# dcy0577/Enhancing-3D-Point-Cloud-Segmentation-Using-Multi-Modal-Fusion-with-2D-Images

Measured on AMD Instinct MI355X. Metric: input points/s through MV-KPConv KPFCNN forward+backward (pyramid + fusion + fwd + bwd + SGD), higher is better.
Workload: dtype f32; 1 GPU; early_fusion_kpfcnn5_sphere19k_x1_per_gpu; views=3, parallelism=dp1, execution=hipGraph[net|chain|enc2d(x2 every 2nd step)+fa], ranks=1, input_lookahead_batches=2, capacity_overflow=False

## Files before the change

enhancing-3d-point-cloud-segmentation-using-multi-modal-fusion-with-2d-images_amd/_lib.py:

```python
import ctypes as C
import os
import re

_HERE = os.path.dirname(os.path.abspath(__file__))
LIB_PATH = os.path.join(_HERE, "libmvkpconv.so")
HEADER_PATH = os.path.join(_HERE, "..", "include", "mvkpconv.h")
SCENE_HEADER_PATH = os.path.join(_HERE, "..", "include", "mvkpconv_scene.h")
TRAIN_HEADER_PATH = os.path.join(_HERE, "..", "include", "mvkpconv_train.h")
SPHERE_HEADER_PATH = os.path.join(_HERE, "..", "include", "mvkpconv_sphere.h")

CTYPES = {"int": C.c_int, "int32_t": C.c_int32, "int64_t": C.c_int64, "float": C.c_float, "double": C.c_double,
          "const char*": C.c_char_p}
_SCALARS = frozenset(t for t in CTYPES if not t.endswith("*"))
_POINTEES = _SCALARS | {"void", "char", "uint8_t", "uint16_t"}
_INTEGER = r"-?(?:0[xX][0-9a-fA-F]+|0|[1-9][0-9]*)"
_DIRECTIVE = re.compile(r"\s*#\s*(?:include\s*<[\w./]+>|ifdef\s+__cplusplus|ifndef\s+\w+_H|endif"
                        r"|define\s+(\w+)(?:\s+(%s))?)\s*" % _INTEGER)
_STRUCT = re.compile(r"typedef\s+struct(?:\s+\w+)?\s*\{([^{}]*)\}\s*(mvk_\w+)\s*;")
_FUNCTION = re.compile(r"([\w\s*]+?)\b(mvk_\w+)\s*\(([^(){};]*)\)\s*;")


def parse_header(text):
    functions, structs, constants = {}, {}, {}

    def fail(pos, what):
        pos += len(text[pos:]) - len(text[pos:].lstrip())
        raise ValueError("mvkpconv.h line %d: %s" % (text.count("\n", 0, pos) + 1, what))

    def canonical(pos, spelling):
        tokens = re.findall(r"\w+|\S", spelling)
        const = tokens[:1] == ["const"]
        base, stars = "".join(tokens[const:const + 1]), tokens[const + 1:]
        if not (stars == [] and not const and base in _SCALARS
                or stars == ["*"] and (base in _POINTEES or base in structs)):
            fail(pos, "unsupported type %r" % " ".join(tokens))
        return "const " * const + base + "*" * len(stars)

    def declarator(pos, spelling):
        m = re.fullmatch(r"(.*[\s*])([A-Za-z_]\w*)\s*", spelling, re.S)
        if not m or m.group(2) == "const" or m.group(2) in _POINTEES:
            fail(pos, "expected '<type> <name>', found %r" % spelling.strip())
        return canonical(pos, m.group(1)), m.group(2)

    text = re.sub(r"/\*.*?\*/|//[^\n]*", lambda m: " " + "\n" * m.group().count("\n"), text, flags=re.S)
    lines = text.split("\n")
    for i, line in enumerate(lines):
        if line.lstrip().startswith("#"):
            m = _DIRECTIVE.fullmatch(line)
            name, value = m.groups() if m else (None, None)
            if not m or (name is not None and (name.startswith("MVK_") != (value is not None) or name in constants)):
                raise ValueError("mvkpconv.h line %d: unsupported preprocessor line %r" % (i + 1, line.strip()))
            if value is not None:
                constants[name] = int(value, 0)
            lines[i] = ""
    text = "\n".join(lines)

    block = re.fullmatch(r'\s*extern\s+"C"\s*\{(.*)\}\s*', text, re.S)
    if not block:
        fail(0, 'expected one extern "C" { ... } block around all declarations')
    pos, end = block.start(1), block.end(1)
    while True:
        pos = re.compile(r"\s*").match(text, pos, end).end()
        if pos == end:
            return functions, structs, constants
        s = _STRUCT.match(text, pos, end)
        f = None if s else _FUNCTION.match(text, pos, end)
        if (s or f) and (s or f).group(2) in functions.keys() | structs.keys():
            fail(pos, "%s is declared twice" % (s or f).group(2))
        if s:
            fields, at = [], s.start(1)
            *statements, tail = s.group(1).split(";")
            if tail.strip() or not statements:
                fail(s.end(1) - len(tail), "struct %s: expected 'type name;' fields" % s.group(2))
            for statement in statements:
                first, *more = statement.split(",")
                ctype, name = declarator(at, first)
                if more and (ctype.endswith("*") or not all(re.fullmatch(r"\s*[A-Za-z_]\w*\s*", n) for n in more)):
                    fail(at, "only scalar fields share a declaration, found %r" % statement.strip())
                fields += [(ctype, n.strip()) for n in [name] + more]
                at += len(statement) + 1
            structs[s.group(2)] = tuple(fields)
        elif f:
            params, at = [], f.start(3)
            for spelling in f.group(3).split(",") if f.group(3).strip() != "void" else ():
                params.append(declarator(at, spelling))
                at += len(spelling) + 1
            functions[f.group(2)] = (canonical(pos, f.group(1)), tuple(params))
        else:
            fail(pos, "neither a function declaration nor a struct typedef: %r" % text[pos:end].split("\n")[0].strip())
        pos = (s or f).end()


def _bind(functions, structs):
    classes = {}

    def ctype(t):
        if t in CTYPES:
            return CTYPES[t]
        assert t.endswith("*"), t
        pointee = t[6 * t.startswith("const "):-1]
        return C.POINTER(classes[pointee]) if pointee in classes else C.c_void_p

    for name, fields in structs.items():
        classes[name] = type("".join(w.capitalize() for w in name.split("_")[1:]), (C.Structure,),
                             {"_fields_": [(n, ctype(t)) for t, n in fields], "__doc__": name + " (include/mvkpconv.h)"})
    return classes, {name: (ctype(ret), [ctype(t) for t, _ in params]) for name, (ret, params) in functions.items()}


def _read_header(path=None, name="mvkpconv.h"):
    path = HEADER_PATH if path is None else path
    if not os.path.exists(path):
        raise RuntimeError(
            "include/%s is not there (%s). The binding reads every prototype of libmvkpconv.so from it -- "
            "run the package from a checkout of the repository; there is no second copy of the C ABI." % (name, path))
    with open(path) as f:
        return f.read()


FUNCTIONS, STRUCTS, CONSTANTS = parse_header(_read_header())
_CLASSES, _PROTOTYPES = _bind(FUNCTIONS, STRUCTS)
EXPORTS = tuple(FUNCTIONS)
ABI_VERSION = CONSTANTS["MVK_ABI_VERSION"]

SCENE_FUNCTIONS, _scene_structs, SCENE_CONSTANTS = parse_header(_read_header(SCENE_HEADER_PATH, "mvkpconv_scene.h"))
if _scene_structs or SCENE_FUNCTIONS.keys() & FUNCTIONS.keys() or SCENE_CONSTANTS.keys() & CONSTANTS.keys():
    raise ValueError("mvkpconv_scene.h: it may declare neither a struct nor a name of mvkpconv.h")
_SCENE_PROTOTYPES = _bind(SCENE_FUNCTIONS, {})[1]

TRAIN_FUNCTIONS, _train_structs, TRAIN_CONSTANTS = parse_header(_read_header(TRAIN_HEADER_PATH, "mvkpconv_train.h"))
if (_train_structs or TRAIN_FUNCTIONS.keys() & (FUNCTIONS.keys() | SCENE_FUNCTIONS.keys())
        or TRAIN_CONSTANTS.keys() & (CONSTANTS.keys() | SCENE_CONSTANTS.keys())):
    raise ValueError("mvkpconv_train.h: it may declare neither a struct nor a name of the other two headers")
_TRAIN_PROTOTYPES = _bind(TRAIN_FUNCTIONS, {})[1]

SPHERE_FUNCTIONS, _sphere_structs, SPHERE_CONSTANTS = parse_header(_read_header(SPHERE_HEADER_PATH, "mvkpconv_sphere.h"))
if (_sphere_structs
        or SPHERE_FUNCTIONS.keys() & (FUNCTIONS.keys() | SCENE_FUNCTIONS.keys() | TRAIN_FUNCTIONS.keys())
        or SPHERE_CONSTANTS.keys() & (CONSTANTS.keys() | SCENE_CONSTANTS.keys() | TRAIN_CONSTANTS.keys())):
    raise ValueError("mvkpconv_sphere.h: it may declare neither a struct nor a name of the other three headers")
_SPHERE_PROTOTYPES = _bind(SPHERE_FUNCTIONS, {})[1]
BnFwdProblem, BnBwdProblem = _CLASSES["mvk_bn_fwd_problem"], _CLASSES["mvk_bn_bwd_problem"]
BnFinish, ATransform = _CLASSES["mvk_bn_finish"], _CLASSES["mvk_a_transform"]
RevList, RegLayer = _CLASSES["mvk_rev_list"], _CLASSES["mvk_reg_layer"]

_lib = None
_owner_pid = None

FORK_MESSAGE = ("the MV-KPConv HIP library was initialised in process %d and is being called from its forked child %d: "
                "a HIP context does not survive fork(). Start DataLoader workers with multiprocessing_context='spawn', "
                "or let the workers emit only stacked points / lengths and build the pyramid "
                "(datasets.common.segmentation_inputs_sphere) in the main process -- see INTEGRATION.md")


def _check_process():
    pid = os.getpid()
    if _owner_pid is not None and pid != _owner_pid:
        raise RuntimeError(FORK_MESSAGE % (_owner_pid, pid))
    try:
        import torch
        if torch.cuda._is_in_bad_fork():
            raise RuntimeError(FORK_MESSAGE % (os.getppid(), pid))
    except (ImportError, AttributeError):
        pass


def lib():
    global _lib, _owner_pid
    _check_process()
    if _lib is None:
        if not os.path.exists(LIB_PATH):
            raise RuntimeError(
                "libmvkpconv.so is not built (%s). Run `python __graft_entry__.py build` -- there is "
                "no CPU fallback for the MV-KPConv hot path." % LIB_PATH)
        l = C.CDLL(LIB_PATH)
        for name, (res, args) in list(_PROTOTYPES.items()) + list(_SCENE_PROTOTYPES.items()) + list(_TRAIN_PROTOTYPES.items()) \
                + list(_SPHERE_PROTOTYPES.items()):
            fn = getattr(l, name)
            fn.restype = res
            fn.argtypes = args
        if l.mvk_abi_version() != ABI_VERSION:
            raise RuntimeError("libmvkpconv.so ABI %d != expected %d; rebuild" % (l.mvk_abi_version(), ABI_VERSION))
        _lib = l
        _owner_pid = os.getpid()
    return _lib


def check(rc):
    if rc != 0:
        raise RuntimeError(lib().mvk_last_error().decode("utf-8", "replace"))
```

enhancing-3d-point-cloud-segmentation-using-multi-modal-fusion-with-2d-images_amd/build.py:

```python
import os
import subprocess
import sys

HERE = os.path.dirname(os.path.abspath(__file__))
CSRC = os.path.join(HERE, "csrc")
OUT = os.path.join(HERE, "libmvkpconv.so")
ARCH = "gfx950"

SOURCES = [
    ("error.cpp", []),
    ("kpconv.hip", []),
    ("gemm.hip", []),
    ("gemm32s.hip", []),
    ("pool.hip", []),
    ("bn.hip", []),
    ("optim.hip", []),
    ("deform.hip", []),
    ("loss.hip", []),
    ("batchpad.hip", []),
    ("revlist.hip", []),
    ("subsample.hip", ["-ffp-contract=off"]),
    ("neighbors.hip", ["-ffp-contract=off"]),
    ("fusion.hip", ["-ffp-contract=off"]),
    ("vote.hip", ["-ffp-contract=off"]),
    ("pn2.hip", ["-ffp-contract=off"]),
    ("chunk.hip", ["-ffp-contract=off"]),
    ("pn2_ordered.hip", ["-ffp-contract=off"]),
    ("pn2_mlp.hip", ["-ffp-contract=off"]),
    ("pn2_rows.hip", ["-ffp-contract=off"]),
    ("scene_inputs.hip", ["-ffp-contract=off"]),
    ("train_inputs.hip", ["-ffp-contract=off"]),
    ("sphere_inputs.hip", ["-ffp-contract=off"]),
]


def _hipcc():
    for c in (os.environ.get("HIPCC"), "/opt/rocm/bin/hipcc", "hipcc"):
        if c and (os.path.isabs(c) and os.path.exists(c) or not os.path.isabs(c)):
            return c
    return "hipcc"


def _stale(target, deps):
    if not os.path.exists(target):
        return True
    t = os.path.getmtime(target)
    return any(os.path.getmtime(d) > t for d in deps if os.path.exists(d))


def build_library(force=False, verbose=False):
    hipcc = _hipcc()
    common = [os.path.join(CSRC, "common.h"), os.path.join(CSRC, "blockscan.h"), os.path.join(CSRC, "compact.h"),
              os.path.join(CSRC, "pn2_rows.h"), os.path.join(CSRC, "unproject.h"), os.path.join(CSRC, "select_frames.h"),
              os.path.join(CSRC, "knn_core.h"), os.path.join(HERE, "..", "include", "mvkpconv_sphere.h"),
              os.path.join(HERE, "..", "include", "mvkpconv.h"), os.path.join(HERE, "..", "include", "mvkpconv_scene.h"),
              os.path.join(HERE, "..", "include", "mvkpconv_train.h"),
              os.path.join(HERE, "..", "include", "mvk_prime_list.h"), os.path.abspath(__file__)]
    objs, jobs = [], []
    for src, extra in SOURCES:
        sp = os.path.join(CSRC, src)
        if not os.path.exists(sp):
            raise FileNotFoundError(sp)
        obj = os.path.join(CSRC, os.path.splitext(src)[0] + ".o")
        if force or _stale(obj, [sp] + common):
            cmd = [hipcc, "--offload-arch=" + ARCH, "-O3", "-std=c++17", "-fPIC", "-c", sp, "-o", obj] + extra
            if src.endswith(".cpp"):
                cmd = [hipcc, "-O2", "-std=c++17", "-fPIC", "-c", sp, "-o", obj]
            jobs.append(cmd)
        objs.append(obj)
    if jobs:
        from concurrent.futures import ThreadPoolExecutor
        n = max(1, min(int(os.environ.get("MVK_BUILD_JOBS", "6")), os.cpu_count() or 1, len(jobs)))

        def run(cmd):
            if verbose:
                print(" ".join(cmd), flush=True)
            subprocess.check_call(cmd)
        with ThreadPoolExecutor(n) as pool:
            list(pool.map(run, jobs))
    if force or _stale(OUT, objs):
        cmd = [hipcc, "--offload-arch=" + ARCH, "-shared", "-fPIC", "-o", OUT] + objs
        if verbose:
            print(" ".join(cmd))
        subprocess.check_call(cmd)
    return OUT


if __name__ == "__main__":
    print(build_library(force="--force" in sys.argv, verbose=True))
```

enhancing-3d-point-cloud-segmentation-using-multi-modal-fusion-with-2d-images_amd/csrc/gemm.hip:

```cpp
#include <stdlib.h>

#include <mutex>
#include <type_traits>

#include "common.h"

namespace {

typedef float f32x4 __attribute__((ext_vector_type(4)));

constexpr int BK = 32;

template <bool CONTIG_K, int ROWS>
struct Tile {
  static constexpr int LD = CONTIG_K ? 40 : ROWS + 4;
  static constexpr int FLOATS = CONTIG_K ? ROWS * 40 : BK * (ROWS + 4);
  static constexpr int NF4 = ROWS * BK / 4;
  static constexpr int NV = (NF4 + 255) / 256;
  static constexpr int IPT = ROWS / 4;
  float4 v[NV];

  __device__ __forceinline__ void transform(const float* __restrict__ xs, int64_t k0, int64_t kbase0, int64_t i0, int64_t imax,
                                            int64_t kmax, int64_t nvalid, float slope, float* __restrict__ out, int64_t ld,
                                            int tid) {
    static_assert(CONTIG_K, "the transform is written for k-contiguous A tiles");
#pragma unroll
    for (int u = 0; u < NV; ++u) {
      const int f = tid + 256 * u;
      if (NF4 % 256 == 0 || f < NF4) {
        const int i = f >> 3, kq = (f & 7) * 4;
        const int64_t gi = i0 + i, gk = k0 + kq;
        const float* t = xs + (gk - kbase0) * 4;
        float e[4] = {v[u].x, v[u].y, v[u].z, v[u].w};
#pragma unroll
        for (int c = 0; c < 4; ++c) {
          const float4 q = *reinterpret_cast<const float4*>(t + 4 * c);
          float z = (e[c] - q.x) * q.y + q.z;
          z = z > 0.f ? z : z * slope;
          e[c] = gi < nvalid ? z : 0.f;
        }
        v[u] = make_float4(e[0], e[1], e[2], e[3]);
        if (out && gi < imax) {
          float* o = out + gi * ld + gk;
          if (gk + 3 < kmax && (ld & 3) == 0)
            *reinterpret_cast<float4*>(o) = v[u];
          else {
#pragma unroll
            for (int c = 0; c < 4; ++c)
              if (gk + c < kmax) o[c] = e[c];
          }
        }
      }
    }
  }

  __device__ __forceinline__ void load(const float* __restrict__ src, int64_t ld, int64_t i0, int64_t imax,
                                       int64_t k0, int64_t kmax, int vec, int tid) {
#pragma unroll
    for (int u = 0; u < NV; ++u) {
      float t[4] = {0.f, 0.f, 0.f, 0.f};
      const int f = tid + 256 * u;
      if (NF4 % 256 == 0 || f < NF4) {
        if (CONTIG_K) {
          const int i = f >> 3, kq = (f & 7) * 4;
          const int64_t gi = i0 + i, gk = k0 + kq;
          if (gi < imax) {
            const float* p = src + gi * ld + gk;
            if (vec == 4 && gk + 3 < kmax) {
              const float4 q = *reinterpret_cast<const float4*>(p);
              t[0] = q.x; t[1] = q.y; t[2] = q.z; t[3] = q.w;
            } else if (vec == 2 && gk + 3 < kmax) {
              const float2 q0 = *reinterpret_cast<const float2*>(p), q1 = *reinterpret_cast<const float2*>(p + 2);
              t[0] = q0.x; t[1] = q0.y; t[2] = q1.x; t[3] = q1.y;
            } else {
#pragma unroll
              for (int e = 0; e < 4; ++e)
                if (gk + e < kmax) t[e] = p[e];
            }
          }
        } else {
          const int k = f / IPT, iq = (f % IPT) * 4;
          const int64_t gk = k0 + k, gi = i0 + iq;
          if (gk < kmax) {
            const float* p = src + gk * ld + gi;
            if (vec == 4 && gi + 3 < imax) {
              const float4 q = *reinterpret_cast<const float4*>(p);
              t[0] = q.x; t[1] = q.y; t[2] = q.z; t[3] = q.w;
            } else if (vec == 2 && gi + 3 < imax) {
              const float2 q0 = *reinterpret_cast<const float2*>(p), q1 = *reinterpret_cast<const float2*>(p + 2);
              t[0] = q0.x; t[1] = q0.y; t[2] = q1.x; t[3] = q1.y;
            } else {
#pragma unroll
              for (int e = 0; e < 4; ++e)
                if (gi + e < imax) t[e] = p[e];
            }
          }
        }
      }
      v[u] = make_float4(t[0], t[1], t[2], t[3]);
    }
  }

  template <int VEC>
  __device__ __forceinline__ void load_fast(const float* __restrict__ src, int64_t ld, int64_t i0, int64_t imax,
                                            int64_t k0, int tid) {
#pragma unroll
    for (int u = 0; u < NV; ++u) {
      int f = tid + 256 * u;
      if (NF4 % 256 != 0) f = f < NF4 ? f : NF4 - 1;
      const float* p;
      if (CONTIG_K) {
        const int i = f >> 3, kq = (f & 7) * 4;
        int64_t gi = i0 + i;
        gi = gi < imax ? gi : imax - 1;
        p = src + gi * ld + (k0 + kq);
      } else {
        const int k = f / IPT, iq = (f % IPT) * 4;
        int64_t gi = i0 + iq;
        gi = gi + 3 < imax ? gi : imax - 4;
        p = src + (k0 + k) * ld + gi;
      }
      if (VEC == 4) {
        const f32x4 q = *reinterpret_cast<const f32x4*>(p);
        v[u] = make_float4(q[0], q[1], q[2], q[3]);
      } else {
        const float2 q0 = *reinterpret_cast<const float2*>(p), q1 = *reinterpret_cast<const float2*>(p + 2);
        v[u] = make_float4(q0.x, q0.y, q1.x, q1.y);
      }
    }
  }

  static __device__ __forceinline__ bool fast_ok(int64_t imax, int vec) {
    return CONTIG_K ? (vec >= 2 && imax >= 1) : (vec == 4 && imax >= 4 && (imax & 3) == 0);
  }

  template <int VEC>
  __device__ __forceinline__ void fetch(const float* __restrict__ src, int64_t ld, int64_t i0, int64_t imax, int64_t k0,
                                        int64_t kmax, int vec, int tid) {
    if (VEC == 0)
      load(src, ld, i0, imax, k0, kmax, vec, tid);
    else
      load_fast<VEC>(src, ld, i0, imax, k0, tid);
  }

  __device__ __forceinline__ void store(float* __restrict__ T, int tid) const {
#pragma unroll
    for (int u = 0; u < NV; ++u) {
      const int f = tid + 256 * u;
      if (NF4 % 256 == 0 || f < NF4) {
        const f32x4 q = {v[u].x, v[u].y, v[u].z, v[u].w};
        if (CONTIG_K) {
          const int i = f >> 3, kq = (f & 7) * 4;
          *reinterpret_cast<f32x4*>(&T[i * LD + kq]) = q;
        } else {
          const int k = f / IPT, iq = (f % IPT) * 4;
          *reinterpret_cast<f32x4*>(&T[k * LD + iq]) = q;
        }
      }
    }
  }

  static __device__ __forceinline__ f32x4 frag(const float* __restrict__ T, int r0, int j, int lane) {
    const int i = lane & 15, g = lane >> 4;
    if (CONTIG_K) {
      return *reinterpret_cast<const f32x4*>(&T[(r0 + i) * LD + 16 * j + 4 * g]);
    } else {
      f32x4 r;
      const float* p = &T[(16 * j + 4 * g) * LD + r0 + i];
      r[0] = p[0];
      r[1] = p[LD];
      r[2] = p[2 * LD];
      r[3] = p[3 * LD];
      return r;
    }
  }
};

struct GemmArgs {
  const float* A;
  const float* B;
  float* C;
  int64_t M, N, Kd, lda, ldb, k_per_split;
  int atomic_out, accumulate, vecA, vecB;
  float* bn_part;
  const int32_t* n_valid;
  const float* bias;
  float act_slope;
  const float* A2;
  const float* B2;
  int64_t Kd2, lda2, ldb2;
  int vecA2, vecB2;
  const void* sc_idx;
  int sc_idx64, sc_c1;
  int64_t sc_stride, sc_ns;
  float* sc_dst;
  float* sc_rest;
  float* det_ws;
  int* det_cnt;
  int det_gx, det_nsplit;
  int seg_shift;
  int64_t seg_extra;
  int* fin_cnt;
  int fin_gy;
  float fin_eps, fin_momentum;
  float* fin_mean;
  float* fin_invstd;
  float* fin_rmean;
  float* fin_rvar;
  long long* fin_nbt;
  const float* ax_mean;
  const float* ax_invstd;
  const float* ax_gamma;
  const float* ax_beta;
  float ax_slope;
  const int32_t* ax_nvalid;
  float* ax_out;
};

constexpr int XF_KMAX = 512;

template <bool TA, bool TB, int PM, int QN, int WM, int WN, bool DUAL = false, bool XF = false>
__device__ __forceinline__ void gemm_body(const GemmArgs& a, const int bx, const int by, const int bz) {
  static_assert(WM * WN == 4, "four waves per workgroup");
  constexpr int TM = 16 * PM * WM, TN = 16 * QN * WN;
  typedef Tile<!TA, TM> TileA;
  typedef Tile<TB, TN> TileB;
  __shared__ __attribute__((aligned(16))) float lds[2 * (TileA::FLOATS + TileB::FLOATS)];
  __shared__ __attribute__((aligned(16))) float xs[XF ? 4 * (XF_KMAX + BK) : 4];
  float* const As = lds;
  float* const Bs = lds + 2 * TileA::FLOATS;
  const int tid = threadIdx.x, lane = tid & 63, wave = tid >> 6;
  const int wm = wave / WN, wn = wave % WN;
  const int64_t m0 = (int64_t)by * TM, n0 = (int64_t)bx * TN;
  const int64_t ktot = DUAL ? a.Kd + a.Kd2 : a.Kd;
  const int64_t kbeg_all = (int64_t)bz * a.k_per_split;
  const int64_t kend_all = kbeg_all + a.k_per_split < ktot ? kbeg_all + a.k_per_split : ktot;

  f32x4 acc[PM][QN];
#pragma unroll
  for (int p = 0; p < PM; ++p)
#pragma unroll
    for (int q = 0; q < QN; ++q) acc[p][q] = (f32x4){0.f, 0.f, 0.f, 0.f};

  int64_t x_nvalid = 0;
  if (XF) {
    for (int k = tid; k < XF_KMAX + BK; k += 256) {
      const int64_t gk = kbeg_all + k;
      float4 q = make_float4(0.f, 0.f, 0.f, 0.f);
      if (gk < a.Kd && k < a.k_per_split + BK) q = make_float4(a.ax_mean[gk], a.ax_invstd[gk] * a.ax_gamma[gk], a.ax_beta[gk], 0.f);
      *reinterpret_cast<float4*>(&xs[4 * k]) = q;
    }
    x_nvalid = a.ax_nvalid ? (int64_t)*a.ax_nvalid : a.M;
    __syncthreads();
  }
  float* const x_out = (XF && bx == 0) ? a.ax_out : nullptr;

  TileA la0, la1;
  TileB lb0, lb1;
  const int ra = wm * 16 * PM, rb = wn * 16 * QN;
  auto compute = [&](const float* __restrict__ Ta, const float* __restrict__ Tb) {
#pragma unroll
    for (int j = 0; j < 2; ++j) {
      f32x4 fa[PM], fb[QN];
#pragma unroll
      for (int p = 0; p < PM; ++p) fa[p] = TileA::frag(Ta, ra + 16 * p, j, lane);
#pragma unroll
      for (int q = 0; q < QN; ++q) fb[q] = TileB::frag(Tb, rb + 16 * q, j, lane);
#pragma unroll
      for (int s = 0; s < 4; ++s)
#pragma unroll
        for (int p = 0; p < PM; ++p)
#pragma unroll
          for (int q = 0; q < QN; ++q)
            acc[p][q] = __builtin_amdgcn_mfma_f32_16x16x4f32(fa[p][s], fb[q][s], acc[p][q], 0, 0, 0);
    }
  };
  float* const A0 = As;
  float* const A1 = As + TileA::FLOATS;
  float* const B0 = Bs;
  float* const B1 = Bs + TileB::FLOATS;
  auto run_range = [&](const float* __restrict__ pA, const int64_t lda, const int vecA, const float* __restrict__ pB,
                       const int64_t ldb, const int vecB, int64_t kbeg, const int64_t kend) {
  auto Bat = [&](const int64_t k) -> const float* {
    return (TB && !DUAL && a.seg_shift >= 0) ? pB + (k >> a.seg_shift) * a.seg_extra : pB;
  };
  auto putA = [&](TileA& la, float* __restrict__ T, const int64_t kt) {
    if constexpr (XF) la.transform(xs, kt, kbeg_all, m0, a.M, a.Kd, x_nvalid, a.ax_slope, x_out, lda, tid);
    la.store(T, tid);
  };
  auto pipeline = [&](auto va, auto vb, const int64_t klim) {
    constexpr int VA = decltype(va)::value, VB = decltype(vb)::value;
    if (kbeg >= klim) return;
    la0.template fetch<VA>(pA, lda, m0, a.M, kbeg, klim, vecA, tid);
    lb0.template fetch<VB>(Bat(kbeg), ldb, n0, a.N, kbeg, klim, vecB, tid);
    if (kbeg + BK < klim) {
      la1.template fetch<VA>(pA, lda, m0, a.M, kbeg + BK, klim, vecA, tid);
      lb1.template fetch<VB>(Bat(kbeg + BK), ldb, n0, a.N, kbeg + BK, klim, vecB, tid);
    }
    putA(la0, A0, kbeg);
    lb0.store(B0, tid);
    __syncthreads();
    for (int64_t k0 = kbeg; k0 < klim; k0 += 2 * BK) {
      if (k0 + 2 * BK < klim) {
        la0.template fetch<VA>(pA, lda, m0, a.M, k0 + 2 * BK, klim, vecA, tid);
        lb0.template fetch<VB>(Bat(k0 + 2 * BK), ldb, n0, a.N, k0 + 2 * BK, klim, vecB, tid);
      }
      compute(A0, B0);
      if (k0 + BK >= klim) break;
      putA(la1, A1, k0 + BK);
      lb1.store(B1, tid);
      __syncthreads();
      if (k0 + 3 * BK < klim) {
        la1.template fetch<VA>(pA, lda, m0, a.M, k0 + 3 * BK, klim, vecA, tid);
        lb1.template fetch<VB>(Bat(k0 + 3 * BK), ldb, n0, a.N, k0 + 3 * BK, klim, vecB, tid);
      }
      compute(A1, B1);
      if (k0 + 2 * BK >= klim) break;
      putA(la0, A0, k0 + 2 * BK);
      lb0.store(B0, tid);
      __syncthreads();
    }
  };
  const bool fastA = TileA::fast_ok(a.M, vecA), fastB = TileB::fast_ok(a.N, vecB);
  const int64_t kfull = kbeg + (kend - kbeg) / BK * BK;
  typedef std::integral_constant<int, 4> I4;
  typedef std::integral_constant<int, 2> I2;
  typedef std::integral_constant<int, 0> I0;
  if (fastA && fastB && vecA == 4 && vecB == 4) {
    pipeline(I4(), I4(), kfull);
  } else if (fastA && fastB && vecA == 2 && vecB == 4) {
    pipeline(I2(), I4(), kfull);
  } else {
    pipeline(I0(), I0(), kend);
    kbeg = kend;
  }
  if (kfull < kend && kbeg < kend) {
    __syncthreads();
    la0.load(pA, lda, m0, a.M, kfull, kend, vecA, tid);
    lb0.load(Bat(kfull), ldb, n0, a.N, kfull, kend, vecB, tid);
    putA(la0, A0, kfull);
    lb0.store(B0, tid);
    __syncthreads();
    compute(A0, B0);
  }
  };
  if (!DUAL) {
    run_range(a.A, a.lda, a.vecA, a.B, a.ldb, a.vecB, kbeg_all, kend_all);
  } else {
    if (kbeg_all < a.Kd) run_range(a.A, a.lda, a.vecA, a.B, a.ldb, a.vecB, kbeg_all, kend_all < a.Kd ? kend_all : a.Kd);
    if (kend_all > a.Kd) {
      if (kbeg_all < a.Kd) __syncthreads();
      run_range(a.A2, a.lda2, a.vecA2, a.B2, a.ldb2, a.vecB2, kbeg_all > a.Kd ? kbeg_all - a.Kd : 0, kend_all - a.Kd);
    }
  }

  if (a.det_ws) {
    constexpr int NB = PM * QN, SLOT = NB * 4 * 256;
    const int64_t tile = (int64_t)by * a.det_gx + bx;
    const __amdgpu_buffer_rsrc_t slots = park_rsrc(a.det_ws + tile * a.det_nsplit * SLOT);
    const uint32_t lane_off = (uint32_t)tid * 16u;
#pragma unroll
    for (int p = 0; p < PM; ++p)
#pragma unroll
      for (int q = 0; q < QN; ++q)
        park_store4(slots, (uint32_t)bz * (SLOT * 4u) + (uint32_t)(p * QN + q) * 4096u + lane_off, acc[p][q]);
    park_wait();
    __syncthreads();
    int* const flag = reinterpret_cast<int*>(lds);
    if (tid == 0) {
      const int old = __hip_atomic_fetch_add(a.det_cnt + tile, 1, __ATOMIC_RELAXED, __HIP_MEMORY_SCOPE_AGENT);
      const int last = old == a.det_nsplit - 1;
      if (last) __hip_atomic_store(a.det_cnt + tile, 0, __ATOMIC_RELAXED, __HIP_MEMORY_SCOPE_AGENT);
      *flag = last;
    }
    __syncthreads();
    const int last = *flag;
    __syncthreads();
    if (!last) return;
#pragma unroll
    for (int p = 0; p < PM; ++p)
#pragma unroll
      for (int q = 0; q < QN; ++q) acc[p][q] = (f32x4){0.f, 0.f, 0.f, 0.f};
    constexpr int ZC = NB >= 8 ? 2 : 4;
    for (int z0 = 0; z0 < a.det_nsplit; z0 += ZC) {
      f32x4 t[ZC][NB];
#pragma unroll
      for (int zz = 0; zz < ZC; ++zz) {
        const int z = z0 + zz < a.det_nsplit ? z0 + zz : a.det_nsplit - 1;
#pragma unroll
        for (int b = 0; b < NB; ++b) t[zz][b] = park_load4(slots, (uint32_t)z * (SLOT * 4u) + (uint32_t)b * 4096u + lane_off);
      }
#pragma unroll
      for (int zz = 0; zz < ZC; ++zz)
        if (z0 + zz < a.det_nsplit) {
#pragma unroll
          for (int p = 0; p < PM; ++p)
#pragma unroll
            for (int q = 0; q < QN; ++q) acc[p][q] += t[zz][p * QN + q];
        }
    }
  }

  const int ci = lane & 15, g4 = (lane >> 4) * 4;
#pragma unroll
  for (int q = 0; q < QN; ++q) {
    const int64_t col = n0 + rb + 16 * q + ci;
    if (col < a.N) {
      const float bq = a.bias ? a.bias[col] : 0.f;
#pragma unroll
      for (int p = 0; p < PM; ++p)
#pragma unroll
        for (int r = 0; r < 4; ++r) {
          const int64_t row = m0 + ra + 16 * p + g4 + r;
          if (row < a.M) {
            if (a.sc_idx) {
              const float v = acc[p][q][r];
              if (col < a.sc_c1) {
                const int j = a.sc_idx64 ? load_idx<true>(a.sc_idx, row * a.sc_stride, a.sc_ns)
                                         : load_idx<false>(a.sc_idx, row * a.sc_stride, a.sc_ns);
                if (j >= 0) atomicAdd(a.sc_dst + (int64_t)j * a.sc_c1 + col, v);
              } else {
                float* c2 = a.sc_rest + row * (a.N - a.sc_c1) + (col - a.sc_c1);
                if (a.atomic_out) atomicAdd(c2, v);
                else *c2 = v;
              }
              continue;
            }
            float* c = a.C + row * a.N + col;
            if (a.atomic_out)
              atomicAdd(c, acc[p][q][r]);
            else if (a.accumulate)
              *c += acc[p][q][r];
            else if (a.bias) {
              const float v = acc[p][q][r] + bq;
              *c = v > 0.f ? v : v * a.act_slope;
            } else
              *c = acc[p][q][r];
          }
        }
    }
  }

  if (a.bn_part) {
    int64_t nv = a.n_valid ? (int64_t)*a.n_valid : a.M;
    nv = nv < a.M ? nv : a.M;
    const int64_t wcnt = nv - (m0 + ra) < 0 ? 0 : (nv - (m0 + ra) > 16 * PM ? 16 * PM : nv - (m0 + ra));
    const int64_t bcnt = nv - m0 < 0 ? 0 : (nv - m0 > TM ? TM : nv - m0);
    const int64_t blk = m0 / TM;
    float* red = lds;
    const __amdgpu_buffer_rsrc_t part_rs = park_rsrc(a.bn_part);
    auto put_part = [&](const int64_t col, const float sum, const float m2) {
      if (a.fin_cnt) {
        park_store1(part_rs, (uint32_t)(((blk * 2) * a.N + col) * 4), sum);
        park_store1(part_rs, (uint32_t)(((blk * 2 + 1) * a.N + col) * 4), m2);
      } else {
        a.bn_part[(blk * 2) * a.N + col] = sum;
        a.bn_part[(blk * 2 + 1) * a.N + col] = m2;
      }
    };
    if (WM > 1) __syncthreads();
    float s[QN], mu[QN];
#pragma unroll
    for (int q = 0; q < QN; ++q) {
      s[q] = 0.f;
#pragma unroll
      for (int p = 0; p < PM; ++p)
#pragma unroll
        for (int r = 0; r < 4; ++r)
          if (16 * p + g4 + r < wcnt) s[q] += acc[p][q][r];
      s[q] += __shfl_xor(s[q], 16);
      s[q] += __shfl_xor(s[q], 32);
      if (WM > 1 && lane < 16) red[wm * TN + rb + 16 * q + ci] = s[q];
    }
    if (WM > 1) {
      __syncthreads();
#pragma unroll
      for (int q = 0; q < QN; ++q) {
        s[q] = 0.f;
#pragma unroll
        for (int w = 0; w < WM; ++w) s[q] += red[w * TN + rb + 16 * q + ci];
      }
    }
#pragma unroll
    for (int q = 0; q < QN; ++q) {
      mu[q] = bcnt > 0 ? s[q] / (float)bcnt : 0.f;
      float m2 = 0.f;
#pragma unroll
      for (int p = 0; p < PM; ++p)
#pragma unroll
        for (int r = 0; r < 4; ++r)
          if (16 * p + g4 + r < wcnt) {
            const float d = acc[p][q][r] - mu[q];
            m2 += d * d;
          }
      m2 += __shfl_xor(m2, 16);
      m2 += __shfl_xor(m2, 32);
      if (WM > 1) {
        if (lane < 16) red[(WM + wm) * TN + rb + 16 * q + ci] = m2;
      } else {
        const int64_t col = n0 + rb + 16 * q + ci;
        if (lane < 16 && col < a.N && m0 < a.M) put_part(col, s[q], m2);
      }
    }
    if (WM > 1) {
      __syncthreads();
      if (wm == 0 && lane < 16) {
#pragma unroll
        for (int q = 0; q < QN; ++q) {
          float m2 = 0.f;
#pragma unroll
          for (int w = 0; w < WM; ++w) m2 += red[(WM + w) * TN + rb + 16 * q + ci];
          const int64_t col = n0 + rb + 16 * q + ci;
          if (col < a.N && m0 < a.M) put_part(col, s[q], m2);
        }
      }
    }
    if (a.fin_cnt) {
      park_wait();
      __syncthreads();
      int* const flag = reinterpret_cast<int*>(lds);
      if (tid == 0) {
        const int old = __hip_atomic_fetch_add(a.fin_cnt + bx, 1, __ATOMIC_RELAXED, __HIP_MEMORY_SCOPE_AGENT);
        const int last = old == a.fin_gy - 1;
        if (last) __hip_atomic_store(a.fin_cnt + bx, 0, __ATOMIC_RELAXED, __HIP_MEMORY_SCOPE_AGENT);
        *flag = last;
      }
      __syncthreads();
      const int last = *flag;
      __syncthreads();
      if (!last) return;
      constexpr int C4 = TN / 4, BL = 256 / C4;
      const int c4 = tid % C4, bl = tid / C4;
      const int64_t col0 = n0 + 4 * c4;
      const int nb = nv > 0 ? (int)((nv + TM - 1) / TM) : 0;
      f32x4 X = {0.f, 0.f, 0.f, 0.f}, Y = {0.f, 0.f, 0.f, 0.f}, ref = {0.f, 0.f, 0.f, 0.f};
      if (col0 < a.N && nb > 0) {
        const float n0f = (float)(nv < TM ? nv : TM);
        ref = park_load4(part_rs, (uint32_t)(col0 * 4));
        ref = ref * (1.f / n0f);
        constexpr int FP = 4;
        for (int i0 = bl; i0 < nb; i0 += FP * BL) {
          f32x4 u[FP], w[FP];
#pragma unroll
          for (int t = 0; t < FP; ++t) {
            const int i = i0 + t * BL < nb ? i0 + t * BL : nb - 1;
            u[t] = park_load4(part_rs, (uint32_t)((((int64_t)i * 2) * a.N + col0) * 4));
            w[t] = park_load4(part_rs, (uint32_t)((((int64_t)i * 2 + 1) * a.N + col0) * 4));
          }
#pragma unroll
          for (int t = 0; t < FP; ++t)
            if (i0 + t * BL < nb) {
              const int64_t left = nv - (int64_t)(i0 + t * BL) * TM;
              const float ni = (float)(left < TM ? left : TM);
              const f32x4 d = u[t] * (1.f / ni) - ref;
              X += u[t];
              Y += w[t] + ni * d * d;
            }
        }
      }
      float* const q1 = lds;
      float* const q2 = lds + 256 * 4;
      *reinterpret_cast<f32x4*>(&q1[bl * TN + 4 * c4]) = X;
      *reinterpret_cast<f32x4*>(&q2[bl * TN + 4 * c4]) = Y;
      float* const qr = lds + 2 * 256 * 4;
      if (bl == 0) *reinterpret_cast<f32x4*>(&qr[4 * c4]) = ref;
      __syncthreads();
      const int64_t col = n0 + tid;
      if (tid < TN && col < a.N) {
        float x = 0.f, y = 0.f;
#pragma unroll 4
        for (int l = 0; l < BL; ++l) {
          x += q1[l * TN + tid];
          y += q2[l * TN + tid];
        }
        float mu = 0.f, var = 0.f, is = 0.f;
        if (nv > 0) {
          mu = x / (float)nv;
          const float dm = mu - qr[tid];
          float M2 = y - (float)nv * dm * dm;
          M2 = M2 > 0.f ? M2 : 0.f;
          var = M2 / (float)nv;
          is = rsqrtf(var + a.fin_eps);
        }
        a.fin_mean[col] = mu;
        a.fin_invstd[col] = is;
        if (a.fin_rmean && nv > 0) {
          const float unbiased = nv > 1 ? var * ((float)nv / (float)(nv - 1)) : var;
          a.fin_rmean[col] = (1.f - a.fin_momentum) * a.fin_rmean[col] + a.fin_momentum * mu;
          a.fin_rvar[col] = (1.f - a.fin_momentum) * a.fin_rvar[col] + a.fin_momentum * unbiased;
        }
      }
      if (a.fin_nbt && bx == 0 && tid == 0) *a.fin_nbt += 1;
    }
  }
}

template <bool TA, bool TB, int PM, int QN, int WM, int WN>
__global__ __launch_bounds__(256) void gemm_f32_mfma(const GemmArgs a) {
  gemm_body<TA, TB, PM, QN, WM, WN>(a, blockIdx.x, blockIdx.y, blockIdx.z);
}

template <bool TB, int PM>
__global__ __launch_bounds__(256) void gemm_f32_mfma_xf(const GemmArgs a) {
  gemm_body<false, TB, PM, 1, 1, 4, false, true>(a, blockIdx.x, blockIdx.y, blockIdx.z);
}

template <bool TA, bool TB, int PM, int QN, int WM, int WN>
__global__ __launch_bounds__(256) void gemm_f32_mfma_pair(const GemmArgs a0, const GemmArgs a1, int gx0, int gz0, int gz1) {
  if ((int)blockIdx.x < gx0) {
    if ((int)blockIdx.z >= gz0) return;
    gemm_body<TA, TB, PM, QN, WM, WN>(a0, blockIdx.x, blockIdx.y, blockIdx.z);
  } else {
    if ((int)blockIdx.z >= gz1) return;
    gemm_body<TA, TB, PM, QN, WM, WN>(a1, blockIdx.x - gx0, blockIdx.y, blockIdx.z);
  }
}

template <bool TA, bool TB, int PM, int QN, int WM, int WN>
__global__ __launch_bounds__(256) void gemm_f32_mfma_dual(const GemmArgs a) {
  gemm_body<TA, TB, PM, QN, WM, WN, true>(a, blockIdx.x, blockIdx.y, blockIdx.z);
}

struct GroupEntry {
  GemmArgs args;
  int gx, gy, gz;
  int wg_begin;
};

template <bool TA, bool TB, int PM, int QN, int WM, int WN>
__global__ __launch_bounds__(256) void gemm_f32_mfma_grouped(const GroupEntry* __restrict__ tab, int n_prob) {
  const int b = blockIdx.x;
  int lo = 0, hi = n_prob - 1;
  while (lo < hi) {
    const int mid = (lo + hi + 1) >> 1;
    if (tab[mid].wg_begin <= b)
      lo = mid;
    else
      hi = mid - 1;
  }
  const GroupEntry& e = tab[lo];
  const int local = b - e.wg_begin;
  const int bx = local % e.gx, by = (local / e.gx) % e.gy, bz = local / (e.gx * e.gy);
  GemmArgs a = e.args;
  a.A = load_global_ptr(&e.args.A);
  a.B = load_global_ptr(&e.args.B);
  a.C = load_global_ptr(&e.args.C);
  a.bn_part = load_global_ptr(&e.args.bn_part);
  a.n_valid = load_global_ptr(&e.args.n_valid);
  a.det_ws = load_global_ptr(&e.args.det_ws);
  a.det_cnt = load_global_ptr(&e.args.det_cnt);
  gemm_body<TA, TB, PM, QN, WM, WN>(a, bx, by, bz);
}


struct Plan {
  int pm, qn, narrow, split;
  int64_t tm() const { return narrow ? 64 * pm : 16 * pm; }
  int64_t tn() const { return narrow ? 16 * qn : 64 * qn; }
};

struct SplitArena {
  float* ws = nullptr;
  int* cnt = nullptr;
  int64_t ws_floats = 0, n_cnt = 0;
  int64_t ws_off = 0, cnt_off = 0;
  int64_t ws_top = 0, cnt_top = 0;
};
SplitArena g_arena;
std::mutex g_arena_mu;

bool ordered_splits() { return g_arena.ws != nullptr; }

int arena_take(hipStream_t st, int64_t tiles, int split, int64_t slot, float** ws, int** cnt) {
  const int64_t need = (tiles * split * slot + 63) / 64 * 64;
  std::lock_guard<std::mutex> lock(g_arena_mu);
  if (need > g_arena.ws_floats || tiles > g_arena.n_cnt) return 1;
  hipStreamCaptureStatus cap = hipStreamCaptureStatusNone;
  if (hipStreamIsCapturing(st, &cap) != hipSuccess) {
    (void)hipGetLastError();
    cap = hipStreamCaptureStatusNone;
  }
  if (cap != hipStreamCaptureStatusNone) {
    if (g_arena.ws_top - need < g_arena.ws_off || g_arena.cnt_top - tiles < g_arena.cnt_off) return 2;
    g_arena.ws_top -= need;
    g_arena.cnt_top -= tiles;
    *ws = g_arena.ws + g_arena.ws_top;
    *cnt = g_arena.cnt + g_arena.cnt_top;
    return 0;
  }
  const int64_t ws_cap = g_arena.ws_top < g_arena.ws_floats / 4 ? g_arena.ws_top : (need > g_arena.ws_floats / 4 ? need : g_arena.ws_floats / 4);
  const int64_t cnt_cap = g_arena.cnt_top < g_arena.n_cnt / 4 ? g_arena.cnt_top : (tiles > g_arena.n_cnt / 4 ? tiles : g_arena.n_cnt / 4);
  if (g_arena.ws_off + need > ws_cap || g_arena.cnt_off + tiles > cnt_cap) {
    if (need > g_arena.ws_top || tiles > g_arena.cnt_top) return 2;
    if (hipDeviceSynchronize() != hipSuccess) return -2;
    g_arena.ws_off = 0;
    g_arena.cnt_off = 0;
  }
  *ws = g_arena.ws + g_arena.ws_off;
  *cnt = g_arena.cnt + g_arena.cnt_off;
  g_arena.ws_off += need;
  g_arena.cnt_off += tiles;
  return 0;
}

const char* arena_error(int rc) {
  return rc == 1 ? "the split-reduction arena is smaller than one product's parking space (MVK_GEMM_ARENA_MB)"
         : rc == 2 ? "the split-reduction arena is used up by the slices captured graphs hold for good: too small for the "
                     "captured steps of this process (MVK_GEMM_ARENA_MB)"
                   : "hipDeviceSynchronize failed while recycling the split-reduction arena";
}

int make_ordered(hipStream_t st, GemmArgs& a, int split, int gx, int64_t gy, int64_t tm, int64_t tn) {
  a.det_ws = nullptr; a.det_cnt = nullptr; a.det_gx = gx; a.det_nsplit = split;
  if (split <= 1 || !ordered_splits()) return 0;
  const int rc = arena_take(st, (int64_t)gx * gy, split, tm * tn, &a.det_ws, &a.det_cnt);
  if (rc != 0) return rc;
  a.atomic_out = 0;
  return 0;
}

#define MVK_ORDERED(call)                                      \
  do {                                                         \
    const int _rc = (call);                                    \
    MVK_REQUIRE(_rc == 0, "gemm: %s", arena_error(_rc));       \
  } while (0)

Plan plan_gemm(int64_t M, int64_t N, int64_t Kd, int split_req, bool want_stats) {
  const int narrow = N <= 32 ? 1 : 0;
  const int pm = narrow ? 1 : (want_stats ? 4 : 2), qn = narrow ? (N <= 16 ? 1 : 2) : 1;
  Plan best{pm, qn, narrow, 1};
  const int64_t tiles = cdiv64(M, best.tm()) * cdiv64(N, best.tn()), ksteps = cdiv64(Kd, BK);
  double best_t = 1e300, t1 = 1e300;
  for (int split = 1; split <= 64; ++split) {
    if (split_req > 0 && split != split_req) continue;
    if (split > 1 && ksteps / split < 4) break;
    const int64_t kt = cdiv64(ksteps, split), wgs = tiles * split;
    double t = (double)cdiv64(wgs, 1280) * (kt * 1500.0 + 3000.0) + (double)wgs * kt * 256.0 * pm * qn / 256.0;
    if (split > 1) t += (double)M * N * split * 4.0 / 2160.0 + 500.0 * split;
    if (split == 1) t1 = t;
    if (t < best_t) {
      best_t = t;
      best.split = split;
    }
  }
  static double bonus = -1.0;
  if (bonus < 0.0) {
    const char* eb = getenv("MVK_GEMM_STATS_BONUS");
    bonus = eb ? atof(eb) : 14000.0;
  }
  if (want_stats && !ordered_splits() && t1 <= best_t + bonus) best.split = 1;
  const char* e = getenv("MVK_GEMM_FORCE");
  if (e) {
    int pm = 0, qn = 0, sp = 0;
    if (sscanf(e, "%d,%d,%d", &pm, &qn, &sp) == 3) {
      if (pm > 0) best.pm = pm;
      if (qn > 0 && !best.narrow) best.qn = qn;
      if (sp > 0 && split_req <= 0) best.split = sp;
    }
  }
  return best;
}

template <bool TA, bool TB, int PM, int QN, int WM, int WN>
void launch_one(dim3 grid, hipStream_t st, const GemmArgs& a) {
  hipLaunchKernelGGL((gemm_f32_mfma<TA, TB, PM, QN, WM, WN>), grid, dim3(256), 0, st, a);
}

template <bool TA, bool TB>
bool launch_cfg(const Plan& p, dim3 grid, hipStream_t st, const GemmArgs& a) {
  if (p.narrow) {
#define NARROW(PMv, QNv) \
  if (p.pm == PMv && p.qn == QNv) return launch_one<TA, TB, PMv, QNv, 4, 1>(grid, st, a), true
    NARROW(1, 1); NARROW(2, 1); NARROW(1, 2); NARROW(2, 2);
#undef NARROW
    return false;
  }
#define WIDE(PMv, QNv) \
  if (p.pm == PMv && p.qn == QNv) return launch_one<TA, TB, PMv, QNv, 1, 4>(grid, st, a), true
  WIDE(1, 1); WIDE(2, 1); WIDE(4, 1); WIDE(5, 1);
  WIDE(1, 2); WIDE(2, 2); WIDE(4, 2);
#undef WIDE
  return false;
}

template <bool TA, bool TB, int PM>
void launch_pair_one(dim3 grid, hipStream_t st, const GemmArgs& a0, const GemmArgs& a1, int gx0, int gz0, int gz1) {
  hipLaunchKernelGGL((gemm_f32_mfma_pair<TA, TB, PM, 1, 1, 4>), grid, dim3(256), 0, st, a0, a1, gx0, gz0, gz1);
}

template <bool TA, bool TB>
bool launch_pair_cfg(const Plan& p, dim3 grid, hipStream_t st, const GemmArgs& a0, const GemmArgs& a1, int gx0, int gz0, int gz1) {
  if (p.qn != 1) return false;
  if (p.pm == 2) return launch_pair_one<TA, TB, 2>(grid, st, a0, a1, gx0, gz0, gz1), true;
  if (p.pm == 4) return launch_pair_one<TA, TB, 4>(grid, st, a0, a1, gx0, gz0, gz1), true;
  return false;
}

void pair_widen(Plan& a, const Plan& b, int64_t Kd) {
  if (a.narrow && !b.narrow && Kd <= 512) {
    a.narrow = 0;
    a.pm = b.pm;
    a.qn = 1;
    a.split = 1;
  }
}

int vec_width(const void* p, int64_t ld) {
  return ((ld % 4 == 0) && ((uintptr_t)p % 16 == 0)) ? 4 : ((ld % 2 == 0) && ((uintptr_t)p % 8 == 0)) ? 2 : 1;
}

struct KSplit { int n; int64_t k_per_split; };
KSplit clamp_split(int64_t Kd, int split) {
  const int64_t ksteps = cdiv64(Kd, BK);
  if (split > ksteps) split = (int)ksteps;
  const int64_t k_per_split = cdiv64(ksteps, split) * BK;
  return {(int)cdiv64(Kd, k_per_split), k_per_split};
}

GemmArgs make_args(const float* A, const float* B, float* C, int64_t M, int64_t N, int64_t Kd, int64_t lda, int64_t ldb,
                   KSplit ks) {
  GemmArgs a{};
  a.A = A; a.B = B; a.C = C; a.M = M; a.N = N; a.Kd = Kd;
  a.lda = lda; a.ldb = ldb; a.vecA = vec_width(A, lda); a.vecB = vec_width(B, ldb);
  a.k_per_split = ks.k_per_split; a.atomic_out = ks.n > 1; a.det_nsplit = ks.n;
  a.act_slope = 1.f; a.ax_slope = 1.f; a.vecA2 = 1; a.vecB2 = 1; a.seg_shift = -1;
  return a;
}

int set_finish(GemmArgs& a, const mvk_bn_finish* fin, int64_t gy) {
  if (!fin) return 0;
  MVK_REQUIRE(a.bn_part != nullptr, "gemm: finished BatchNorm statistics need the statistics epilogue (plan: stat rows 0)");
  MVK_REQUIRE(fin->counters && fin->mean && fin->invstd && a.N % 4 == 0 && (uintptr_t)a.bn_part % 16 == 0,
              "gemm: finished statistics need counters, mean, invstd and a channel count that is a multiple of 4");
  MVK_REQUIRE((fin->running_mean == nullptr) == (fin->running_var == nullptr), "gemm: running_mean and running_var go together");
  a.fin_cnt = fin->counters; a.fin_gy = (int)gy; a.fin_eps = fin->eps; a.fin_momentum = fin->momentum;
  a.fin_mean = fin->mean; a.fin_invstd = fin->invstd; a.fin_rmean = fin->running_mean; a.fin_rvar = fin->running_var;
  a.fin_nbt = (long long*)fin->num_batches_tracked;
  return 0;
}

struct ScatterOut {
  const void* idx;
  int idx64, c1;
  int64_t stride, ns;
  float* dst;
  float* rest;
};

struct GemmOpts {
  int accumulate = 0, split_k = 0;
  float* bn_part = nullptr;
  const int32_t* n_valid = nullptr;
  const float* bias = nullptr;
  float act_slope = 1.f;
  const ScatterOut* scatter = nullptr;
  int seg_shift = -1;
  int64_t seg_extra = 0, ldb = 0, lda = 0;
  const mvk_bn_finish* fin = nullptr;
  const mvk_a_transform* ax = nullptr;
};

int gemm_run(const float* A, const float* B, float* C, int64_t M, int64_t N, int64_t Kd, int transA, int transB,
             const GemmOpts& o, void* stream) {
  MVK_REQUIRE(M >= 0 && N >= 0 && Kd >= 0, "gemm: negative size");
  if (M == 0 || N == 0) return 0;
  hipStream_t st = (hipStream_t)stream;
  MVK_REQUIRE(!(o.bn_part && (o.accumulate || Kd == 0)), "gemm: BatchNorm statistics need a plain store of a non-empty product");
  if (Kd == 0) {
    if (!o.accumulate && o.split_k <= 1) MVK_CHECK_HIP(hipMemsetAsync(C, 0, sizeof(float) * M * N, st));
    return 0;
  }
  MVK_REQUIRE(!(o.bn_part && o.split_k > 1 && !ordered_splits()), "gemm: BatchNorm statistics need an unsplit (or ordered) reduction");
  const Plan p = plan_gemm(M, N, Kd, (o.bn_part && !ordered_splits()) ? 1 : (o.split_k > 0 ? o.split_k : 0), o.bn_part != nullptr);
  const KSplit ks = clamp_split(Kd, p.split);
  const int64_t lda = o.lda > 0 ? o.lda : (transA ? M : Kd);
  if (cdiv64(M, p.tm()) >= 65536) {
    MVK_REQUIRE(!o.bn_part && !o.fin && !o.ax && !o.scatter && o.seg_shift < 0 && ks.n < 65536, "gemm: grid too large");
    constexpr int64_t CHUNK = 15 * 65536;
    GemmOpts oc = o;
    oc.split_k = ks.n;
    oc.lda = lda;
    for (int64_t m0 = 0; m0 < M; m0 += CHUNK) {
      const int64_t mc = M - m0 < CHUNK ? M - m0 : CHUNK;
      if (int e = gemm_run(A + (transA ? m0 : m0 * lda), B, C + m0 * N, mc, N, Kd, transA, transB, oc, stream)) return e;
    }
    return 0;
  }
  GemmArgs a = make_args(A, B, C, M, N, Kd, lda, o.ldb > 0 ? o.ldb : (transB ? Kd : N), ks);
  if (o.seg_shift >= 0) {
    a.ldb = (int64_t)1 << o.seg_shift;
    a.vecB = ((uintptr_t)B % 16 == 0 && o.seg_extra % 4 == 0) ? 4 : 1;
  }
  a.accumulate = o.accumulate; a.bn_part = o.bn_part; a.n_valid = o.n_valid; a.bias = o.bias; a.act_slope = o.act_slope;
  a.seg_shift = o.seg_shift; a.seg_extra = o.seg_extra;
  if (o.scatter) {
    a.sc_idx = o.scatter->idx; a.sc_idx64 = o.scatter->idx64; a.sc_c1 = o.scatter->c1; a.sc_stride = o.scatter->stride;
    a.sc_ns = o.scatter->ns; a.sc_dst = o.scatter->dst; a.sc_rest = o.scatter->rest;
  }
  MVK_REQUIRE(cdiv64(M, p.tm()) < 65536 && ks.n < 65536, "gemm: grid too large");
  dim3 grid((unsigned)cdiv64(N, p.tn()), (unsigned)cdiv64(M, p.tm()), (unsigned)ks.n);
  MVK_ORDERED(make_ordered(st, a, ks.n, (int)grid.x, grid.y, p.tm(), p.tn()));
  MVK_REQUIRE(!(o.bn_part && ks.n > 1 && !a.det_ws), "gemm: BatchNorm statistics of a split product need the ordered reduction");
  if (int e = set_finish(a, o.fin, grid.y)) return e;
  if (const mvk_a_transform* ax = o.ax) {
    MVK_REQUIRE(!transA && transB && !p.narrow && p.qn == 1 && (p.pm == 2 || p.pm == 4) && ks.k_per_split <= XF_KMAX && !o.scatter &&
                    o.seg_shift < 0 && ax->mean && ax->invstd && ax->gamma && ax->beta && ax->slope > 0.f,
                "gemm: the operand transform needs an NT product of more than 32 columns with k-ranges <= %d", XF_KMAX);
    a.ax_mean = ax->mean; a.ax_invstd = ax->invstd; a.ax_gamma = ax->gamma; a.ax_beta = ax->beta; a.ax_slope = ax->slope;
    a.ax_nvalid = ax->n_valid; a.ax_out = ax->out;
    if (p.pm == 2) hipLaunchKernelGGL((gemm_f32_mfma_xf<true, 2>), grid, dim3(256), 0, st, a);
    else hipLaunchKernelGGL((gemm_f32_mfma_xf<true, 4>), grid, dim3(256), 0, st, a);
    MVK_CHECK_HIP(hipGetLastError());
    return 0;
  }
  bool ok;
  if (!transA && !transB) ok = launch_cfg<false, false>(p, grid, st, a);
  else if (!transA && transB) ok = launch_cfg<false, true>(p, grid, st, a);
  else if (transA && !transB) ok = launch_cfg<true, false>(p, grid, st, a);
  else ok = launch_cfg<true, true>(p, grid, st, a);
  MVK_REQUIRE(ok, "gemm: no kernel for plan pm=%d qn=%d narrow=%d", p.pm, p.qn, p.narrow);
  MVK_CHECK_HIP(hipGetLastError());
  return 0;
}

int gemm_pair_run(const float* A, const float* B0, const float* B1, float* C0, float* C1, int64_t M, int64_t N0, int64_t N1,
                  int64_t Kd, int transB, int want_stats, float* bn_part0, float* bn_part1, const int32_t* n_valid,
                  const mvk_bn_finish* fin0, const mvk_bn_finish* fin1, void* stream) {
  MVK_REQUIRE(M > 0 && N0 > 0 && N1 > 0 && Kd > 0, "gemm pair: empty product");
  Plan p0 = plan_gemm(M, N0, Kd, 0, want_stats != 0), p1 = plan_gemm(M, N1, Kd, 0, want_stats != 0);
  pair_widen(p0, p1, Kd);
  MVK_REQUIRE(!p0.narrow && !p1.narrow && p0.pm == p1.pm && p0.qn == 1 && p1.qn == 1 && (p0.pm == 2 || p0.pm == 4),
              "gemm pair: the two products do not share a tile shape (ask mvk_gemm_f32_pair_plan first)");
  hipStream_t st = (hipStream_t)stream;
  const bool ord = ordered_splits();
  const KSplit s0 = clamp_split(Kd, p0.split), s1 = clamp_split(Kd, p1.split);
  GemmArgs a0 = make_args(A, B0, C0, M, N0, Kd, Kd, transB ? Kd : N0, s0);
  GemmArgs a1 = make_args(A, B1, C1, M, N1, Kd, Kd, transB ? Kd : N1, s1);
  a0.bn_part = (want_stats && (p0.split == 1 || ord)) ? bn_part0 : nullptr;
  a1.bn_part = (want_stats && (p1.split == 1 || ord)) ? bn_part1 : nullptr;
  a0.n_valid = a1.n_valid = n_valid;
  const int64_t tm = p0.tm(), tn = p0.tn(), gy = cdiv64(M, tm);
  MVK_REQUIRE(gy < 65536 && s0.n < 65536 && s1.n < 65536, "gemm: grid too large");
  const int gx0 = (int)cdiv64(N0, tn), gx1 = (int)cdiv64(N1, tn);
  MVK_ORDERED(make_ordered(st, a0, s0.n, gx0, gy, tm, tn));
  MVK_ORDERED(make_ordered(st, a1, s1.n, gx1, gy, tm, tn));
  MVK_REQUIRE(ord || ((s0.n == 1 || !a0.bn_part) && (s1.n == 1 || !a1.bn_part)), "gemm pair: statistics of a split product");
  if (int e = set_finish(a0, fin0, gy)) return e;
  if (int e = set_finish(a1, fin1, gy)) return e;
  dim3 grid((unsigned)(gx0 + gx1), (unsigned)gy, (unsigned)(s0.n > s1.n ? s0.n : s1.n));
  const bool ok = transB ? launch_pair_cfg<false, true>(p0, grid, st, a0, a1, gx0, s0.n, s1.n)
                         : launch_pair_cfg<false, false>(p0, grid, st, a0, a1, gx0, s0.n, s1.n);
  MVK_REQUIRE(ok, "gemm pair: no kernel for plan pm=%d", p0.pm);
  MVK_CHECK_HIP(hipGetLastError());
  return 0;
}

}

bool mvk_internal_arena_take(void* stream, int64_t floats, int64_t counters, float** ws, int** cnt) {
  if (!ordered_splits() || floats < 0 || counters < 0) return false;
  return arena_take((hipStream_t)stream, counters > 0 ? counters : 1, 1, cdiv64(floats, counters > 0 ? counters : 1), ws, cnt) == 0;
}

extern "C" int mvk_gemm_split_arena(void* ws, int64_t ws_bytes, void* counters, int64_t n_counters) {
  MVK_REQUIRE((ws == nullptr) == (counters == nullptr) && ws_bytes >= 0 && n_counters >= 0, "gemm arena: bad arguments");
  MVK_REQUIRE(ws == nullptr || (ws_bytes >= (1 << 20) && n_counters >= 4096 && (uintptr_t)ws % 256 == 0),
              "gemm arena: at least 1 MB of 256-byte aligned slots and 4096 counters");
  std::lock_guard<std::mutex> lock(g_arena_mu);
  g_arena.ws = (float*)ws;
  g_arena.cnt = (int*)counters;
  g_arena.ws_floats = ws ? ws_bytes / 4 : 0;
  g_arena.n_cnt = ws ? n_counters : 0;
  g_arena.ws_off = 0;
  g_arena.cnt_off = 0;
  g_arena.ws_top = g_arena.ws_floats;
  g_arena.cnt_top = g_arena.n_cnt;
  return 0;
}

extern "C" int mvk_gemm_split_ordered(void) { return ordered_splits() ? 1 : 0; }

extern "C" int mvk_gemm_f32_dual_plan(int64_t M, int64_t N, int64_t Kd, int64_t Kd2, int* out_split) {
  MVK_REQUIRE(M >= 0 && N >= 0 && Kd >= 0 && Kd2 >= 0 && out_split, "gemm dual plan: bad arguments");
  *out_split = 0;
  if (M == 0 || N == 0 || Kd == 0 || Kd2 == 0 || Kd % BK != 0) return 0;
  const Plan p = plan_gemm(M, N, Kd + Kd2, 0, false);
  if (p.narrow || p.qn != 1 || p.pm != 2) return 0;
  *out_split = clamp_split(Kd + Kd2, p.split).n;
  return 0;
}

extern "C" int mvk_gemm_f32_dual(const float* A, const float* B, const float* A2, const float* B2, float* C, int64_t M,
                                 int64_t N, int64_t Kd, int64_t Kd2, void* stream) {
  MVK_REQUIRE(M > 0 && N > 0 && Kd > 0 && Kd2 > 0 && Kd % BK == 0, "gemm dual: unsupported shape (ask mvk_gemm_f32_dual_plan)");
  const Plan p = plan_gemm(M, N, Kd + Kd2, 0, false);
  MVK_REQUIRE(!p.narrow && p.qn == 1 && p.pm == 2, "gemm dual: unsupported shape (ask mvk_gemm_f32_dual_plan)");
  hipStream_t st = (hipStream_t)stream;
  const KSplit ks = clamp_split(Kd + Kd2, p.split);
  GemmArgs a = make_args(A, B, C, M, N, Kd, Kd, N, ks);
  a.A2 = A2; a.B2 = B2; a.Kd2 = Kd2; a.lda2 = Kd2; a.ldb2 = N;
  a.vecA2 = vec_width(A2, a.lda2);
  a.vecB2 = vec_width(B2, a.ldb2);
  MVK_REQUIRE(cdiv64(M, 32) < 65536 && ks.n < 65536, "gemm: grid too large");
  dim3 grid((unsigned)cdiv64(N, 64), (unsigned)cdiv64(M, 32), (unsigned)ks.n);
  MVK_ORDERED(make_ordered(st, a, ks.n, (int)grid.x, grid.y, 32, 64));
  hipLaunchKernelGGL((gemm_f32_mfma_dual<false, false, 2, 1, 1, 4>), grid, dim3(256), 0, st, a);
  MVK_CHECK_HIP(hipGetLastError());
  return 0;
}

extern "C" int mvk_gemm_f32_pair_plan(int64_t M, int64_t N0, int64_t N1, int64_t Kd, int want_stats, int* out ) {
  MVK_REQUIRE(M >= 0 && N0 >= 0 && N1 >= 0 && Kd >= 0 && out, "gemm pair plan: bad arguments");
  for (int i = 0; i < 5; ++i) out[i] = 0;
  if (M == 0 || N0 == 0 || N1 == 0 || Kd == 0) return 0;
  Plan p0 = plan_gemm(M, N0, Kd, 0, want_stats != 0), p1 = plan_gemm(M, N1, Kd, 0, want_stats != 0);
  pair_widen(p0, p1, Kd);
  if (p0.narrow || p1.narrow || p0.pm != p1.pm || p0.qn != 1 || p1.qn != 1 || (p0.pm != 2 && p0.pm != 4)) return 0;
  out[0] = 1;
  out[1] = p0.split;
  out[2] = p1.split;
  out[3] = (want_stats && (p0.split == 1 || ordered_splits())) ? (int)p0.tm() : 0;
  out[4] = (want_stats && (p1.split == 1 || ordered_splits())) ? (int)p1.tm() : 0;
  return 0;
}

extern "C" int mvk_gemm_f32_pair(const float* A, const float* B0, const float* B1, float* C0, float* C1, int64_t M,
                                 int64_t N0, int64_t N1, int64_t Kd, int transB, int want_stats, float* bn_part0,
                                 float* bn_part1, const int32_t* n_valid, void* stream) {
  return gemm_pair_run(A, B0, B1, C0, C1, M, N0, N1, Kd, transB, want_stats, bn_part0, bn_part1, n_valid, nullptr, nullptr, stream);
}
extern "C" int mvk_gemm_f32_pair_bn(const float* A, const float* B0, const float* B1, float* C0, float* C1, int64_t M,
                                    int64_t N0, int64_t N1, int64_t Kd, int transB, float* bn_part0, float* bn_part1,
                                    const int32_t* n_valid, const mvk_bn_finish* fin0, const mvk_bn_finish* fin1, void* stream) {
  return gemm_pair_run(A, B0, B1, C0, C1, M, N0, N1, Kd, transB, 1, bn_part0, bn_part1, n_valid, fin0, fin1, stream);
}

extern "C" int mvk_gemm_f32_plan(int64_t M, int64_t N, int64_t Kd, int split_k, int want_stats, int* out_split,
                                 int* out_stat_rows) {
  MVK_REQUIRE(M >= 0 && N >= 0 && Kd >= 0 && out_split && out_stat_rows, "gemm plan: bad arguments");
  if (M == 0 || N == 0 || Kd == 0) {
    *out_split = 1;
    *out_stat_rows = 0;
    return 0;
  }
  const Plan p = plan_gemm(M, N, Kd, split_k > 0 ? split_k : 0, want_stats != 0);
  *out_split = p.split;
  *out_stat_rows = (want_stats && (p.split == 1 || ordered_splits())) ? (int)p.tm() : 0;
  return 0;
}

extern "C" int mvk_gemm_f32_ex(const float* A, const float* B, float* C, int64_t M, int64_t N, int64_t Kd,
                               int transA, int transB, int accumulate, int split_k, float* bn_part,
                               const int32_t* n_valid, void* stream) {
  GemmOpts o; o.accumulate = accumulate; o.split_k = split_k; o.bn_part = bn_part; o.n_valid = n_valid;
  return gemm_run(A, B, C, M, N, Kd, transA, transB, o, stream);
}

extern "C" int mvk_gemm_f32_bn(const float* A, const float* B, float* C, int64_t M, int64_t N, int64_t Kd, int transB,
                               float* bn_part, const int32_t* n_valid, const mvk_bn_finish* fin, const mvk_a_transform* ax,
                               void* stream) {
  MVK_REQUIRE(M > 0 && N > 0 && Kd > 0, "gemm bn: empty product");
  GemmOpts o; o.bn_part = bn_part; o.n_valid = n_valid; o.fin = fin; o.ax = ax;
  return gemm_run(A, B, C, M, N, Kd, 0, transB, o, stream);
}

extern "C" int mvk_gemm_f32_bias_act(const float* A, const float* B, float* C, int64_t M, int64_t N, int64_t Kd, int transB,
                                     const float* bias, float slope, void* stream) {
  MVK_REQUIRE(bias != nullptr && slope > 0.f && Kd > 0, "gemm bias_act: bias, a positive slope and a non-empty product");
  GemmOpts o; o.split_k = 1; o.bias = bias; o.act_slope = slope;
  return gemm_run(A, B, C, M, N, Kd, 0, transB, o, stream);
}

extern "C" int mvk_gemm_f32_kp_transposed(const float* A, const float* W, float* dx, int64_t M, int K, int Cin, int Cout,
                                          void* stream) {
  MVK_REQUIRE(K >= 1 && Cin >= 1 && Cout >= BK && (Cout & (Cout - 1)) == 0, "gemm kp_transposed: Cout must be a power of two >= 32");
  int shift = 0;
  while ((1 << shift) < Cout) ++shift;
  GemmOpts o; o.seg_shift = shift; o.seg_extra = (int64_t)Cin * Cout - Cout;
  return gemm_run(A, W, dx, M, Cin, (int64_t)K * Cout, 0, 1, o, stream);
}

extern "C" int mvk_gemm_f32_ldb(const float* A, const float* B, float* C, int64_t M, int64_t N, int64_t Kd, int64_t ldb,
                                void* stream) {
  MVK_REQUIRE(ldb >= N, "gemm ldb: ldb < N");
  GemmOpts o; o.ldb = ldb;
  return gemm_run(A, B, C, M, N, Kd, 0, 0, o, stream);
}

extern "C" int mvk_gemm_f32_scatter_cat(const float* A, const float* B, int64_t M, int64_t N, int64_t Kd, const void* idx,
                                        int idx64, int64_t idx_stride, int64_t Ns, int c1, float* d_x, float* d_skip,
                                        void* stream) {
  MVK_REQUIRE(idx && d_x && d_skip && c1 > 0 && c1 < N && Kd > 0 && Ns >= 0 && idx_stride >= 1, "gemm scatter_cat: bad arguments");
  const ScatterOut sc{idx, idx64, c1, idx_stride, Ns, d_x, d_skip};
  GemmOpts o; o.scatter = &sc;
  return gemm_run(A, B, d_skip , M, N, Kd, 0, 0, o, stream);
}

struct MvkGemmProblem {
  const float* A;
  const float* B;
  float* C;
  int64_t M, N, Kd;
};

extern "C" int64_t mvk_gemm_group_entry_bytes(void) { return (int64_t)sizeof(GroupEntry); }

constexpr int GROUP_KTILES_MIN = 16, GROUP_KTILES_MAX = 96;

int group_wide_pm() {
  static const int v = getenv("MVK_DW_WIDE_PM") ? atoi(getenv("MVK_DW_WIDE_PM")) : 4;
  return v == 2 || v == 8 ? v : 4;
}

int group_ktiles_env() {
  static const int v = getenv("MVK_DW_GROUP_KTILES") ? atoi(getenv("MVK_DW_GROUP_KTILES")) : -1;
  return v;
}

int grouped_split_at(int64_t M, int64_t N, int64_t Kd, int ktiles) {
  if (ktiles <= 0) return plan_gemm(M, N, Kd, 0, false).split;
  int64_t split = cdiv64(cdiv64(Kd, BK), ktiles);
  return (int)(split > 64 ? 64 : (split < 1 ? 1 : split));
}

extern "C" int mvk_gemm_f32_tn_grouped_split(int64_t M, int64_t N, int64_t Kd) {
  const int e = group_ktiles_env();
  return grouped_split_at(M, N, Kd, e >= 0 ? e : GROUP_KTILES_MIN);
}

extern "C" int mvk_gemm_f32_tn_grouped_plan(const void* problems, int n, void* table_host, int* n_narrow,
                                            int64_t* wgs_narrow, int64_t* wgs_wide, int32_t* splits ,
                                            void* stream ) {
  MVK_REQUIRE(n >= 0 && problems && table_host && n_narrow && wgs_narrow && wgs_wide && splits, "grouped gemm: bad arguments");
  const MvkGemmProblem* pr = (const MvkGemmProblem*)problems;
  GroupEntry* tab = (GroupEntry*)table_host;
  int nn = 0;
  for (int i = 0; i < n; ++i) nn += pr[i].N <= 32 ? 1 : 0;
  int64_t wn = 0, ww = 0;
  int in = 0, iw = nn;
  int ktiles = group_ktiles_env();
  if (ktiles < 0) {
    double units = 0.0;
    for (int i = 0; i < n; ++i)
      units += (double)cdiv64(pr[i].M, pr[i].N <= 32 ? 64 : 16 * group_wide_pm()) * cdiv64(pr[i].N, pr[i].N <= 32 ? 32 : 64) * cdiv64(pr[i].Kd, BK);
    const double t = units / 8000.0;
    ktiles = t < GROUP_KTILES_MIN ? GROUP_KTILES_MIN : (t > GROUP_KTILES_MAX ? GROUP_KTILES_MAX : (int)t);
  }
  for (int i = 0; i < n; ++i) {
    const MvkGemmProblem& q = pr[i];
    MVK_REQUIRE(q.M > 0 && q.N > 0 && q.Kd > 0 && q.A && q.B && q.C, "grouped gemm: empty problem %d", i);
    const bool narrow = q.N <= 32;
    MVK_REQUIRE(!narrow || q.N > 16, "grouped gemm: outputs of <= 16 columns are not grouped");
    const KSplit ks = clamp_split(q.Kd, grouped_split_at(q.M, q.N, q.Kd, ktiles));
    const int split = ks.n;
    GroupEntry e{};
    e.args = make_args(q.A, q.B, q.C, q.M, q.N, q.Kd, q.M, q.N, ks);
    const int64_t tm = narrow ? 64 : 16 * group_wide_pm(), tn = narrow ? 32 : 64;
    e.gx = (int)cdiv64(q.N, tn);
    e.gy = (int)cdiv64(q.M, tm);
    e.gz = split;
    MVK_ORDERED(make_ordered((hipStream_t)stream, e.args, split, e.gx, e.gy, tm, tn));
    const int64_t wgs = (int64_t)e.gx * e.gy * e.gz;
    if (narrow) {
      e.wg_begin = (int)wn;
      wn += wgs;
      tab[in++] = e;
    } else {
      e.wg_begin = (int)ww;
      ww += wgs;
      tab[iw++] = e;
    }
    splits[i] = split;
  }
  MVK_REQUIRE(wn < (1ll << 31) && ww < (1ll << 31), "grouped gemm: grid too large");
  *n_narrow = nn;
  *wgs_narrow = wn;
  *wgs_wide = ww;
  return 0;
}

extern "C" int mvk_gemm_f32_tn_grouped(const void* table_dev, int n, int n_narrow, int64_t wgs_narrow, int64_t wgs_wide,
                                       void* stream) {
  MVK_REQUIRE(n >= 0 && n_narrow >= 0 && n_narrow <= n, "grouped gemm: bad counts");
  hipStream_t st = (hipStream_t)stream;
  const GroupEntry* tab = (const GroupEntry*)table_dev;
  if (n_narrow > 0 && wgs_narrow > 0)
    hipLaunchKernelGGL((gemm_f32_mfma_grouped<true, false, 1, 2, 4, 1>), dim3((unsigned)wgs_narrow), dim3(256), 0, st, tab,
                       n_narrow);
  if (n - n_narrow > 0 && wgs_wide > 0) {
    if (group_wide_pm() == 4)
      hipLaunchKernelGGL((gemm_f32_mfma_grouped<true, false, 4, 1, 1, 4>), dim3((unsigned)wgs_wide), dim3(256), 0, st,
                         tab + n_narrow, n - n_narrow);
    else if (group_wide_pm() == 8)
      hipLaunchKernelGGL((gemm_f32_mfma_grouped<true, false, 8, 1, 1, 4>), dim3((unsigned)wgs_wide), dim3(256), 0, st,
                         tab + n_narrow, n - n_narrow);
    else
      hipLaunchKernelGGL((gemm_f32_mfma_grouped<true, false, 2, 1, 1, 4>), dim3((unsigned)wgs_wide), dim3(256), 0, st,
                         tab + n_narrow, n - n_narrow);
  }
  MVK_CHECK_HIP(hipGetLastError());
  return 0;
}

extern "C" int mvk_gemm_f32(const float* A, const float* B, float* C, int64_t M, int64_t N, int64_t Kd, int transA,
                            int transB, int accumulate, int split_k, void* stream) {
  return mvk_gemm_f32_ex(A, B, C, M, N, Kd, transA, transB, accumulate, split_k, nullptr, nullptr, stream);
}
```

enhancing-3d-point-cloud-segmentation-using-multi-modal-fusion-with-2d-images_amd/ops.py:

```python
import collections
import os
import ctypes as C

import weakref

import torch

from ._lib import lib, check, CONSTANTS, SCENE_CONSTANTS, TRAIN_CONSTANTS, SPHERE_CONSTANTS

INFLUENCE = {k[len("MVK_INFL_"):].lower(): v for k, v in CONSTANTS.items() if k.startswith("MVK_INFL_")}
AGGREGATION = {k[len("MVK_AGG_"):].lower(): v for k, v in CONSTANTS.items() if k.startswith("MVK_AGG_")}


def _p(t):
    return C.c_void_p(t.data_ptr()) if t is not None else None


def _stream():
    return C.c_void_p(torch.cuda.current_stream().cuda_stream)


def _dev(*ts):
    for t in ts:
        if t is not None and not t.is_cuda:
# ... 138 lines not shown
    e = getattr(t, "_mvk_bn_stats", None)
    return e if e is None or isinstance(e, BnStats) else BnStats(*e)


def bn_finished(t):
    return getattr(bn_stats_of(t), "finished", None) is not None


def _finishable(bn):
    return BN_FOLD and bn is not None and bn.training and _SYNC_BN["group"] is None and bn.num_features % 4 == 0


def _fin_counters(bn, device):
    c = getattr(bn, "_mvk_fin_counters", None)
    if c is None or c.device != device:
        if torch.cuda.is_current_stream_capturing():
            raise RuntimeError("ops: the finish counters of a BatchNorm do not exist yet and cannot be created inside a "
                               "graph capture; run one eager step first")
        c = torch.zeros(128, dtype=torch.int32, device=device)
        torch.cuda.current_stream(device).synchronize()
        bn._mvk_fin_counters = c
    return c


def _fin_struct(bn, N, device):
    from ._lib import BnFinish
    if bn.num_features != N:
        raise RuntimeError("ops: the BatchNorm handed to a product has %d channels, the product %d columns" % (bn.num_features, N))
    mean = torch.empty(N, device=device, dtype=torch.float32)
    invstd = torch.empty(N, device=device, dtype=torch.float32)
    track = bn.track_running_stats and bn.running_mean is not None
    fin = BnFinish(_p(_fin_counters(bn, device)), float(bn.eps), float(bn.momentum if bn.momentum is not None else 0.0),
                   _p(mean), _p(invstd), _p(bn.running_mean) if track else None, _p(bn.running_var) if track else None,
                   _p(bn.num_batches_tracked) if track else None)
    return fin, (mean, invstd)


def gemm(A, B, transA=False, transB=False, out=None, accumulate=False, split_k=None, keep=False, stats_n_valid=None):
    out, st = _product(A, B, transA=transA, transB=transB, out=out, accumulate=accumulate, split_k=split_k, keep=keep,
                       stats_n_valid=stats_n_valid)
    if stats_n_valid is None:
        return out
    return out, (st[:2] if st is not None else None)


def _product(A, B, *, transA=False, transB=False, out=None, accumulate=False, split_k=None, keep=False,
             stats_n_valid=None, finish=None, a_transform=None):
    _dev(A, B)
    A, B = _f32c(A), _f32c(B)
    M, Kd = (A.shape[1], A.shape[0]) if transA else (A.shape[0], A.shape[1])
    N = B.shape[0] if transB else B.shape[1]
    assert (B.shape[1] if transB else B.shape[0]) == Kd, "gemm: inner dimensions differ"
    ax = a_transform
    if ax is not None and (ax["lazy"].data_ptr() != A.data_ptr() or transA or not transB or out is not None or accumulate
                           or M == 0):
        raise RuntimeError("ops: a product with an operand transform takes the lazy tensor as A, W as transposed B and "
                           "an output of its own")
    if M == 0 or N == 0 or Kd == 0:
        return (out.zero_() if out is not None else torch.zeros((M, N), device=A.device, dtype=torch.float32)), None
    split_arena_prepare(A.device)
    stats_ok = stats_n_valid is not None and out is None and not accumulate and M <= _STATS_EPILOGUE_ROWS
    if finish is None and ax is None:
        stats_ok = stats_ok and M > bn_single_launch_rows(N)
    split, rows = gemm_plan(M, N, Kd, split_k, stats_ok)
    if out is None:
        out = _split_out((M, N), A.device, split, keep)
    elif split > 1 and not accumulate and A.device.index not in _SPLIT_ARENA:
        out.zero_()
    part =torch.empty(((M + rows - 1) // rows, 2, N), device=A.device, dtype=torch.float32) if rows > 0 else None
    fin = done = None
    if finish is not None and part is not None and not transA and split_k is None:
        fin, done = _fin_struct(finish, N, A.device)
    if fin is not None or ax is not None:
        xf = None
        if ax is not None:
            from ._lib import ATransform
            xf = ATransform(_p(ax["mean"]), _p(ax["invstd"]), _p(ax["gamma"]), _p(ax["beta"]), float(ax["slope"]),
                            _p(ax["n_valid"]), _p(ax["lazy"]))
            A = ax["raw"]
        check(lib().mvk_gemm_f32_bn(_p(A), _p(B), _p(out), M, N, Kd, int(transB), _p(part),
                                    _p(stats_n_valid) if part is not None else None,
                                    C.byref(fin) if fin is not None else None, C.byref(xf) if xf is not None else None,
                                    _stream()))
    else:
        check(lib().mvk_gemm_f32_ex(_p(A), _p(B), _p(out), M, N, Kd, int(transA), int(transB), int(accumulate),
                                    int(split), _p(part), _p(stats_n_valid) if part is not None else None, _stream()))
    return out, (BnStats(part, rows, done) if part is not None else None)


def gemm_f32_stream_plan(M, N, Kd):
    out = (C.c_int64 * 4)()
    check(lib().mvk_gemm_f32_stream_plan(int(M), int(N), int(Kd), out))
    return bool(out[0]), int(out[1]), int(out[2]), int(out[3])


def _slack_floats(t):
    return t.untyped_storage().nbytes() // 4 - t.storage_offset() - t.numel()


def gemm_f32_stream(A, B, stats_n_valid=None):
    _dev(A, B, stats_n_valid)
    A, B = _f32c(A), _f32c(B)
    M, Kd = A.shape
    N = B.shape[1]
    ok, tiles, wgs, need = gemm_f32_stream_plan(M, N, Kd)
    if not ok or B.shape[0] != Kd:
        raise RuntimeError("gemm_f32_stream: unsupported shape %d x %d x %d" % (M, N, Kd))
    y = torch.empty((M, N), device=A.device, dtype=torch.float32)
    part = torch.empty((wgs, 2, N), device=A.device, dtype=torch.float32) if stats_n_valid is not None else None
    check(lib().mvk_gemm_f32_stream(_p(A), _slack_floats(A), _p(B), _p(y), M, N, Kd, _p(stats_n_valid), _p(part), _stream()))
    return y, ((part, 16 * tiles) if part is not None else None)


_PROF = {"on": False, "rec": [], "gemm": []}


def profile_reset(enabled):
    _PROF["on"] = bool(enabled)
    _PROF["rec"] = []
    _PROF["gemm"] = []
    _PROF["h_eff"] = {}


def _timing_events():
    torch.cuda._sleep(200000)
    e0, e1 = torch.cuda.Event(enable_timing=True), torch.cuda.Event(enable_timing=True)
    e0.record()
    return e0, e1


def profile_collect_contraction():
    torch.cuda.synchronize()
    out = {}
    for key, e0, e1 in _PROF["gemm"]:
        r = out.setdefault(key, {"launches": 0, "total_ms": 0.0, "flops_per_launch": 2.0 * key[0] * key[1] * key[2]})
        r["launches"] += 1
        r["total_ms"] += e0.elapsed_time(e1)
    return out


def _gather_kernel_label(Nq, Ns, H, Cin, deform, fast=True):
    p = kpconv_gather_plan(Nq, Ns, H, Cin, 4, deform)
    if fast and p["mfma"]:
        return "kpconv_gather_mfma<T=%d>(1 point per wave)" % p["rows_per_batch"]
    return "kpconv_lane_channel<fwd,deform>" if deform else "kpconv_lane_channel<fwd>"


def profile_collect(h_eff=None):
    torch.cuda.synchronize()
    out = {}
    for key, e0, e1 in _PROF["rec"]:
        r = out.setdefault(key, {"launches": 0, "total_ms": 0.0, "each_ms": []})
        r["launches"] += 1
        t = e0.elapsed_time(e1)
        r["total_ms"] += t
        r["each_ms"].append(t)
    for key, r in out.items():
        name, Nq, Ns, H, Cin, K = key
        he = _PROF.get("h_eff", {}).get((Nq, Ns, H)) if name.endswith("[dx]") else None
        if he is None:
            he = (h_eff or {}).get((Nq, Ns, H), H)
        sx = 4
        r["bytes_per_launch"] = Nq * he * (Cin * sx + 12 + 4) + Nq * 12 + Nq * K * Cin * sx
        r["kernel"] = name
        r["shape"] = {"Nq": Nq, "Ns": Ns, "H": H, "H_eff": he, "Cin": Cin, "K": K}
    return out


def kpconv_gather(q, s, idx, x, kp, extent, influence="linear", aggregation="sum", offsets=None,
                  want_min_d2=False, order=None, tag=None):
    _dev(q, s, idx, x, kp, offsets, order)
    if order is not None and (order.dtype != torch.int32 or order.shape != (q.shape[0],) or not order.is_contiguous()):
        raise RuntimeError("kpconv_gather: order must be a contiguous int32 tensor of Nq entries")
    q, s, x, kp = _f32c(q), _f32c(s), _f32c(x), _f32c(kp)
    idx, i64 = _idx(idx)
    Nq, Ns, H, Cin, K = q.shape[0], s.shape[0], idx.shape[1] if idx.dim() == 2 else 0, x.shape[1], kp.shape[0]
    if x.shape[0] != Ns:
        raise RuntimeError("kpconv: features and support points differ in length")
    A = torch.empty(Nq * K * Cin + 64, device=q.device, dtype=torch.float32)[:Nq * K * Cin].view(Nq, K, Cin)
    min_d2 = min_arg = None
    if offsets is not None:
        offsets = _f32c(offsets)
        if want_min_d2:
            min_d2 = torch.empty((Nq, K), device=q.device, dtype=torch.float32)
            min_arg = torch.empty((Nq, K), device=q.device, dtype=torch.int32)
    if _PROF["on"]:
        e0, e1 = _timing_events()
    check(lib().mvk_kpconv_gather_fwd_ordered(_p(q), Nq, _p(s), Ns, _p(idx), i64, H, _p(x), Cin, _p(kp), K,
                                              float(extent), INFLUENCE[influence], AGGREGATION[aggregation],
                                              _p(offsets), _p(min_d2), _p(min_arg), _p(A), _p(order), _stream()))
    if _PROF["on"]:
        e1.record()
        name = _gather_kernel_label(Nq, Ns, H, Cin, offsets is not None, (influence, aggregation) == ("linear", "sum"))
        if tag:
            name += tag
            _PROF.setdefault("h_eff", {})[(Nq, Ns, H)] = float((idx < Ns).sum().item()) / max(Nq, 1)
        _PROF["rec"].append(((name, Nq, Ns, H, Cin, K), e0, e1))
    if min_d2 is not None:
        min_d2._mvk_min_arg = min_arg
    return A, min_d2


def kpconv_scatter(q, s, idx, dA, kp, extent, influence="linear", aggregation="sum", x=None,
                   offsets=None, g_min_d2=None, min_arg=None):
    _dev(q, s, idx, dA, kp)
    q, s, dA, kp = _f32c(q), _f32c(s), _f32c(dA), _f32c(kp)
    idx, i64 = _idx(idx)
    Nq, Ns, H, K, Cin = q.shape[0], s.shape[0], idx.shape[1], kp.shape[0], dA.shape[2]
    dx = _zeros((Ns, Cin), q.device)
    d_off = None
    if offsets is not None:
        offsets, x = _f32c(offsets), _f32c(x)
        d_off = (torch.zeros if (Nq == 0 or H == 0) else torch.empty)((Nq, K, 3), device=q.device, dtype=torch.float32)
        if g_min_d2 is not None:
            g_min_d2 = _f32c(g_min_d2)
            if min_arg is None:
                raise RuntimeError("kpconv_scatter: the min_d2 gradient needs the forward's arg-min columns")
    check(lib().mvk_kpconv_scatter_bwd(_p(q), Nq, _p(s), Ns, _p(idx), i64, H, Cin, _p(kp), K, float(extent),
                                       INFLUENCE[influence], AGGREGATION[aggregation], _p(dA), _p(dx),
                                       _p(x), _p(offsets), _p(g_min_d2), _p(min_arg), _p(d_off), _stream()))
    return dx, d_off


def kpconv_deform_doff(q, s, idx, x, kp, extent, offsets, dA, g_min_d2=None, min_arg=None):
    _dev(q, s, idx, x, kp, offsets, dA, g_min_d2, min_arg)
    q, s, x, kp, offsets, dA = _f32c(q), _f32c(s), _f32c(x), _f32c(kp), _f32c(offsets), _f32c(dA)
    idx, i64 = _idx(idx)
    Nq, Ns, H, K, Cin = q.shape[0], s.shape[0], idx.shape[1], kp.shape[0], dA.shape[2]
    if Nq == 0 or H == 0:
        return torch.zeros((Nq, K, 3), device=q.device, dtype=torch.float32)
    d_off = torch.empty((Nq, K, 3), device=q.device, dtype=torch.float32)
    if g_min_d2 is not None:
        g_min_d2 = _f32c(g_min_d2)
        if min_arg is None:
            raise RuntimeError("kpconv_deform_doff: the min_d2 gradient needs the forward's arg-min columns")
    check(lib().mvk_kpconv_deform_doff(_p(q), Nq, _p(s), Ns, _p(idx), i64, H, _p(x), Cin, _p(kp), K, float(extent),
                                       INFLUENCE["linear"], _p(offsets), _p(dA), _p(g_min_d2), _p(min_arg), _p(d_off),
                                       _stream()))
    return d_off


def kpconv_gather_rev_deform(s, q, rev, g, kp, extent, offsets, modulations=None, order=None):
    _dev(s, q, rev, g, kp, offsets, modulations, order)
    s, q, g, kp, offsets = _f32c(s), _f32c(q), _f32c(g), _f32c(kp), _f32c(offsets)
    if modulations is not None:
        modulations = _f32c(modulations)
    rev, r64 = _idx(rev)
    Ns, Nq, Hr, Cc, K = s.shape[0], q.shape[0], rev.shape[1], g.shape[1], kp.shape[0]
    if rev.shape[0] != Ns or g.shape[0] != Nq or offsets.shape != (Nq, K, 3):
        raise RuntimeError("kpconv_gather_rev_deform: rev [Ns,Hr], g [Nq,C] and offsets [Nq,K,3] expected")
    A2 = torch.empty(Ns * K * Cc + 64, device=s.device, dtype=torch.float32)[:Ns * K * Cc].view(Ns, K, Cc)
    check(lib().mvk_kpconv_gather_rev_deform(_p(s), Ns, _p(q), Nq, _p(rev), r64, Hr, _p(g), Cc, _p(kp), K, float(extent),
                                             _p(offsets), _p(modulations), _p(A2), _p(order), _stream()))
    return A2


_DEFER = {"on": False, "items": [], "leaves": set(), "slots": None, "eager": 0}
_DW_MAX = 512


def _defer_slots(device):
    if _DEFER["slots"] is None:
        nb = _DW_MAX * int(lib().mvk_gemm_group_entry_bytes())
        _DEFER["slots"] = [{"host": torch.empty(nb, dtype=torch.uint8).pin_memory(),
                            "dev": torch.empty(nb, dtype=torch.uint8, device=device), "event": None} for _ in range(34)]
    return _DEFER["slots"]


def capture_table_slots_left(device):
    return max(0, len(_defer_slots(device)) - 2)


class defer_weight_grads:

    def __init__(self, flush=True):
        self.flush = bool(flush)
        self.items = []

    def __enter__(self):
        _DEFER.update(on=True, items=[], leaves=set())
        return self

    def __exit__(self, *exc):
        try:
            if exc[0] is None:
                if self.flush:
                    _flush_deferred()
                else:
                    self.items = _DEFER["items"]
        finally:
            _DEFER.update(on=False, items=[], leaves=set())
        return False

    def take(self):
        items, self.items = self.items, []
        return items


def flush_deferred(items, stream=None):
    if not items:
        return
    if stream is None or stream == torch.cuda.current_stream():
        return _flush_deferred(items)
    for (A, B, _, _, _) in items:
        A.record_stream(stream)
        B.record_stream(stream)
    with torch.cuda.stream(stream):
        _flush_deferred(items)


_HAS_USE_COUNT = hasattr(torch._C, "_storage_Use_Count")


def _storage_use_count(storage):
    return torch._C._storage_Use_Count(storage._cdata)


def _flush_deferred(items=None):
    if items is None:
        items = _DEFER["items"]
    if not items:
        return
    import numpy as np
    dev = items[0][0].device
    n = len(items)
    prob = np.zeros(n, dtype=np.dtype([("A", "<u8"), ("B", "<u8"), ("C", "<u8"), ("M", "<i8"), ("N", "<i8"), ("Kd", "<i8")]))
    for i, (A, B, out_ptr, _, storage) in enumerate(items):
        if _storage_use_count(storage) < 2:
            raise RuntimeError("defer_weight_grads: a deferred weight-gradient result (%d x %d) was consumed before the "
                               "grouped launch computed it; was the backward run on parameters that already hold a "
                               ".grad, or with hooks that copy gradients? Run it without the scope (MVK_DEFER_DW=0)"
                               % (A.shape[1], B.shape[1]))
        prob[i] = (A.data_ptr(), B.data_ptr(), out_ptr, A.shape[1], B.shape[1], A.shape[0])
    slots = _defer_slots(dev)
    if torch.cuda.is_current_stream_capturing():
        if len(slots) <= 2:
            raise RuntimeError("defer_weight_grads: out of pre-pinned table slots for graph captures")
        slot = slots.pop()
        _DEFER.setdefault("captured", []).append(slot)
    else:
        slot = slots[_DEFER["eager"] % 2]
        _DEFER["eager"] += 1
        if slot["event"] is not None:
            slot["event"].synchronize()
    nn, wn, ww = C.c_int(0), C.c_int64(0), C.c_int64(0)
    splits = np.zeros(n, np.int32)
    check(lib().mvk_gemm_f32_tn_grouped_plan(prob.ctypes.data_as(C.c_void_p), n, C.c_void_p(slot["host"].data_ptr()),
                                             C.byref(nn), C.byref(wn), C.byref(ww), splits.ctypes.data_as(C.c_void_p),
                                             _stream()))
    for i, item in enumerate(items):
        if splits[i] > 1 and not item[3] and not lib().mvk_gemm_split_ordered():
            raise RuntimeError("defer_weight_grads: the grouped plan splits a product whose output was not zero-initialised")
    nb = n * int(lib().mvk_gemm_group_entry_bytes())
    slot["dev"][:nb].copy_(slot["host"][:nb], non_blocking=True)
    check(lib().mvk_gemm_f32_tn_grouped(C.c_void_p(slot["dev"].data_ptr()), n, nn.value, wn.value, ww.value, _stream()))
    if not torch.cuda.is_current_stream_capturing():
        ev = torch.cuda.Event()
        ev.record()
        slot["event"] = ev


def _accumulate_in_place_ok(t):
    if _DEFER["on"] and _DEFER["items"]:
        st = t.untyped_storage().data_ptr()
        for it in _DEFER["items"]:
            if it[0].untyped_storage().data_ptr() == st or it[1].untyped_storage().data_ptr() == st:
                return False
    return True


def _dw_gemm(A, B, transB=False, target=None):
    leaf = target if (target is not None and target.is_leaf) else None
    if _DEFER["on"] and leaf is not None:
        if id(leaf) in _DEFER["leaves"]:
            raise RuntimeError("defer_weight_grads: the same parameter receives two weight gradients inside one scope "
                               "(shared weights): run this backward without the scope (MVK_DEFER_DW=0)")
        if leaf.grad is not None:
            return gemm(A, B, transA=True, transB=transB)
    if _DEFER["on"] and _HAS_USE_COUNT and not transB and A.is_cuda and B.shape[1] > 16 and len(_DEFER["items"]) < _DW_MAX \
            and A.shape[0] > 0 and A.shape[1] > 0:
        A, B = _f32c(A), _f32c(B)
        split_arena_prepare(A.device)
        zeroed = lib().mvk_gemm_f32_tn_grouped_split(A.shape[1], B.shape[1], A.shape[0]) > 1 \
            and not lib().mvk_gemm_split_ordered()
        out = (_zeros((A.shape[1], B.shape[1]), A.device) if zeroed
               else torch.empty((A.shape[1], B.shape[1]), device=A.device, dtype=torch.float32))
        _DEFER["items"].append((A, B, out.data_ptr(), zeroed, out.untyped_storage()))
        if leaf is not None:
            _DEFER["leaves"].add(id(leaf))
        return out
    return gemm(A, B, transA=True, transB=transB)



class _KPConvFn(torch.autograd.Function):

    @staticmethod
    def forward(ctx, q, s, idx, x, kp, W, offsets, modulations, extent, influence, aggregation, stats_n_valid=None,
                order=None, rev=None, rev_order=None, finish=None):
        K, Cin, Cout = W.shape
        deform = offsets is not None
        A, min_d2 = kpconv_gather(q, s, idx, x, kp, extent, influence, aggregation, offsets, want_min_d2=deform,
                                  order=order)
        ctx.rev = (rev, rev_order)
        Am = A * modulations.unsqueeze(2) if modulations is not None else A
        if _PROF["on"]:
            e0, e1 = _timing_events()
        st = None
        if _contraction_streams(Am, q.shape[0], K * Cin, Cout):
            y, st = gemm_f32_stream(Am.view(-1, K * Cin), W.reshape(K * Cin, Cout), stats_n_valid)
            st = BnStats(*st) if st is not None else None
        else:
            y, st = _product(Am.view(-1, K * Cin), W.reshape(K * Cin, Cout), stats_n_valid=stats_n_valid, finish=finish)
        if _PROF["on"]:
            e1.record()
            _PROF["gemm"].append(((q.shape[0], K * Cin, Cout), e0, e1))
        ctx.save_for_backward(q, s, idx, x, kp, W, A, offsets, modulations)
        ctx.min_arg = getattr(min_d2, "_mvk_min_arg", None)
        ctx.cfg = (extent, influence, aggregation)
        if st is not None:
            ctx.mark_non_differentiable(st.partials)
        ctx.set_materialize_grads(False)
        return y, min_d2, st

    @staticmethod
    def backward(ctx, gy, g_min_d2, g_st=None):
        q, s, idx, x, kp, W, A, offsets, modulations = ctx.saved_tensors
        extent, influence, aggregation = ctx.cfg
        K, Cin, Cout = W.shape
        Nq = q.shape[0]
        if gy is None:
            gy = torch.zeros((Nq, Cout), device=q.device, dtype=torch.float32)
        gy = _f32c(gy)
        Am = A * modulations.unsqueeze(2) if modulations is not None else A
        dW = dx = d_off = d_mod = None
        if ctx.needs_input_grad[5]:
            dW = _dw_gemm(Am.view(Nq, K * Cin), gy, target=W).view(K, Cin, Cout)
        need_dA = ctx.needs_input_grad[3] or (offsets is not None)
        rev, rev_order = ctx.rev
        gather_form = (need_dA and rev is not None and REVERSE_DX and rev.shape[0] >= s.shape[0] and Cout >= 5
                       and influence == "linear" and aggregation == "sum")
        if gather_form and rev.shape[0] != s.shape[0]:
            rev = rev[:s.shape[0]]
        if gather_form and offsets is None and modulations is None:
            A2, _ = kpconv_gather(s, q, rev, gy, _neg_kernel_points(kp), extent, influence, aggregation, order=rev_order,
                                  tag="[dx]")
            dx = kp_transposed_contraction(A2, W)
        elif need_dA:
            dAm = gemm(gy, W.reshape(K * Cin, Cout), transB=True).view(Nq, K, Cin)
            if modulations is not None:
                if ctx.needs_input_grad[7]:
                    d_mod = (dAm * A).sum(dim=2)
                dA = dAm * modulations.unsqueeze(2)
            else:
                dA = dAm
            if gather_form and offsets is not None:
                d_off = kpconv_deform_doff(q, s, idx, x, kp, extent, offsets, dA, g_min_d2, ctx.min_arg)
                if ctx.needs_input_grad[3]:
                    A2 = kpconv_gather_rev_deform(s, q, rev, gy, kp, extent, offsets, modulations, order=rev_order)
                    dx = kp_transposed_contraction(A2, W)
            else:
                dx, d_off = kpconv_scatter(q, s, idx, dA, kp, extent, influence, aggregation, x=x,
                                           offsets=offsets,
                                           g_min_d2=g_min_d2 if offsets is not None else None, min_arg=ctx.min_arg)
        return None, None, None, dx, None, dW, d_off, d_mod, None, None, None, None, None, None, None, None


def _contraction_streams(A, M, Kd, N):
    if M <= 0:
        return False
    ok, _, _, need = gemm_f32_stream_plan(M, N, Kd)
    return ok and A.is_contiguous() and _slack_floats(A) >= need


def kpconv(q, s, idx, x, kp, W, extent, influence="linear", aggregation="sum", offsets=None, modulations=None,
           stats_n_valid=None, order=None, rev=None, rev_order=None, bn=None):
    if rev is not None and (rev.dtype != torch.int32 or rev.dim() != 2 or not rev.is_contiguous()):
        raise RuntimeError("kpconv: rev must be a contiguous int32 [Ns, Hr] matrix (ops.reverse_neighbors)")
    if influence not in INFLUENCE:
        raise ValueError("Unknown influence function type (config.KP_influence)")
    if aggregation not in AGGREGATION:
        raise ValueError("Unknown convolution mode. Should be 'closest' or 'sum'")
    y, min_d2, st = _KPConvFn.apply(q, s, idx, x, kp, W, offsets, modulations, float(extent), influence, aggregation,
                                    stats_n_valid, order, rev, rev_order,
                                    bn if stats_n_valid is not None and _finishable(bn) else None)
    if st is not None:
        y._mvk_bn_stats = st
    return y, min_d2



class _DeformRegFn(torch.autograd.Function):

    @staticmethod
    def forward(ctx, min_d2, deformed_kp, n_valid, extent, repulse_extent, power):
        _dev(min_d2, deformed_kp, n_valid)
        min_d2, dkp = _f32c(min_d2), _f32c(deformed_kp)
        N, K = min_d2.shape
        loss = _zeros((1,), min_d2.device)
        d_min = torch.empty_like(min_d2)
        d_dkp = torch.empty_like(dkp)
        check(lib().mvk_deform_regularizer(_p(min_d2), _p(dkp), _p(n_valid), N, K, float(extent), float(repulse_extent),
                                           float(power), _p(loss), _p(d_min), _p(d_dkp), _stream()))
        ctx.save_for_backward(d_min, d_dkp)
        return loss.reshape(())

    @staticmethod
    def backward(ctx, g):
        d_min, d_dkp = ctx.saved_tensors
        return d_min * g, d_dkp * g, None, None, None, None


class _DeformOperandsFn(torch.autograd.Function):

    @staticmethod
    def forward(ctx, raw, bias, kernel_points, extent, modulated):
        _dev(raw, bias, kernel_points)
        raw, bias, kp = _f32c(raw), _f32c(bias), _f32c(kernel_points)
        N, D = raw.shape
        K = kp.shape[0]
        if D != (4 if modulated else 3) * K or bias.numel() != D:
            raise RuntimeError("deform operands: the inner convolution must deliver %d columns" % ((4 if modulated else 3) * K))
        feat = torch.empty_like(raw)
        offsets = torch.empty((N, K, 3), device=raw.device, dtype=torch.float32)
        dkp = torch.empty_like(offsets)
        mod = torch.empty((N, K), device=raw.device, dtype=torch.float32) if modulated else None
        check(lib().mvk_deform_operands_fwd(_p(raw), _p(bias), _p(kp), N, K, int(bool(modulated)), float(extent), _p(feat),
                                            _p(offsets), _p(dkp), _p(mod), _stream()))
        ctx.save_for_backward(mod)
        ctx.cfg = (N, K, D, float(extent), bool(modulated))
        ctx.set_materialize_grads(False)
        return feat, offsets, dkp, mod

    @staticmethod
    def backward(ctx, g_feat, g_off, g_dkp, g_mod):
        (mod,) = ctx.saved_tensors
        N, K, D, extent, modulated = ctx.cfg
        dev = (mod if mod is not None else next(g for g in (g_feat, g_off, g_dkp, g_mod) if g is not None)).device
        gs = [None if g is None else _f32c(g) for g in (g_off, g_dkp, g_mod, g_feat)]
        d_raw = torch.empty((N, D), device=dev, dtype=torch.float32)
        d_bias = _zeros((D,), dev)
        check(lib().mvk_deform_operands_bwd(_p(gs[0]), _p(gs[1]), _p(gs[2]), _p(mod), _p(gs[3]), N, K, int(modulated), extent,
                                            _p(d_raw), _p(d_bias), _stream()))
        return d_raw, d_bias, None, None, None


def deform_operands(raw, bias, kernel_points, extent, modulated=False):
    return _DeformOperandsFn.apply(raw, bias, kernel_points, extent, modulated)


def _reg_many(cfgs, ts, grads, loss, gscale):
    from ._lib import RegLayer
    by_k = {}
    for i, (extent, repulse, power, nv) in enumerate(cfgs):
        m, d = ts[2 * i], ts[2 * i + 1]
        L = RegLayer(_p(m), _p(d), _p(nv), _p(grads[2 * i]) if grads else None, _p(grads[2 * i + 1]) if grads else None,
                     m.shape[0], float(extent), float(repulse), float(power))
        by_k.setdefault(int(m.shape[1]), []).append(L)
    for K, layers in by_k.items():
        for b in range(0, len(layers), REG_MANY):
            part = layers[b:b + REG_MANY]
            arr = (RegLayer * len(part))(*part)
            check(lib().mvk_deform_regularizer_many(arr, len(part), K, _p(loss), _p(gscale), _stream()))


class _DeformRegAllFn(torch.autograd.Function):

    @staticmethod
    def forward(ctx, cfgs, *tensors):
        ts = [_f32c(t) for t in tensors]
        _dev(*ts)
        loss = _zeros((1,), ts[0].device)
        _reg_many(cfgs, ts, None, loss, None)
        ctx.save_for_backward(*ts)
        ctx.cfgs = cfgs
        return loss.reshape(())

    @staticmethod
    def backward(ctx, g):
        ts = ctx.saved_tensors
        g = _f32c(g).reshape(1)
        grads = [torch.empty_like(t) for t in ts]
        _reg_many(ctx.cfgs, ts, grads, None, g)
        return (None, *grads)


def deform_regularizer_all(layers):
    layers = [l for l in layers if l[0].shape[0] > 0]
    if not layers:
        return None
    cfgs = [(l[2], l[3], l[4], l[5]) for l in layers]
    flat = []
    for l in layers:
        flat += [l[0], l[1]]
    return _DeformRegAllFn.apply(cfgs, *flat)


def deform_regularizer(min_d2, deformed_kp, extent, repulse_extent, power=1.0, n_valid=None):
    return _DeformRegFn.apply(min_d2, deformed_kp, n_valid, extent, repulse_extent, power)



_ROW_COUNTS = {}


def set_row_counts(mapping):
    _ROW_COUNTS.clear()
    if mapping:
        _ROW_COUNTS.update(mapping)


def row_count_for(rows):
    return _ROW_COUNTS.get(int(rows))


_COUNT_TABLE = {}
_COUNT_TABLE_ROWS = 1 << 22
_BIG_COUNTS = {}


def full_count(rows, device):
    rows = int(rows)
    t = _COUNT_TABLE.get(device.index)
    if t is None:
        if torch.cuda.is_current_stream_capturing():
            raise RuntimeError("ops.full_count: the constant row-count table does not exist yet and cannot be created "
                               "inside a graph capture; run one eager step first or call ops.full_count_prepare(device)")
        t = torch.arange(_COUNT_TABLE_ROWS, dtype=torch.int32, device=device)
        torch.cuda.current_stream(device).synchronize()
        _COUNT_TABLE[device.index] = t
    if 0 <= rows < _COUNT_TABLE_ROWS:
        return t[rows:rows + 1]
    key = (rows, device.index)
    w = _BIG_COUNTS.get(key)
    if w is None:
        if torch.cuda.is_current_stream_capturing():
            raise RuntimeError("ops.full_count: %d rows lie beyond the constant table; request this count once outside "
                               "the capture" % rows)
        w = torch.full((1,), rows, dtype=torch.int32, device=device)
        torch.cuda.current_stream(device).synchronize()
        _BIG_COUNTS[key] = w
    return w


def full_count_prepare(device):
    full_count(0, torch.device(device))


def _bn_fwd_problem(who, x, n_valid, gamma, beta, running_mean, running_var, cfg, nbt, addend, ext):
    R, D = x.shape
    y = torch.empty_like(x)
    ext_part, ext_rows, fin = ext if ext is not None else (None, 0, None)
    if ext_part is not None and (ext_part.shape[2] != D or ext_part.shape[0] != (R + ext_rows - 1) // ext_rows):
        raise RuntimeError("%s: the statistics partials do not belong to this tensor" % who)
    scratch = None
    if fin is not None:
        mean, invstd = fin
        running_mean = running_var = nbt = ext_part = None
        ext_rows = -1
    else:
        mean = torch.empty(D, device=x.device, dtype=torch.float32)
        invstd = torch.empty(D, device=x.device, dtype=torch.float32)
        if ext_part is None:
            scratch = torch.empty(((R + 63) // 64) * 2 * D, device=x.device, dtype=torch.float32)
    eps, momentum, slope = cfg
    args = (_p(x), _p(n_valid), R, D, _p(gamma), _p(beta), float(eps), float(momentum), float(slope), _p(running_mean),
            _p(running_var), _p(mean), _p(invstd), _p(scratch), _p(y), _p(nbt), _p(addend), _p(ext_part), int(ext_rows))
    return args, y, mean, invstd, scratch


def _bn_bwd_problem(x, g, n_valid, gamma, beta, mean, invstd, slope, yout):
    g = _f32c(g)
    R, D = x.shape
    dgb = torch.empty(2 * D, device=x.device, dtype=torch.float32)
    scratch = torch.empty(((R + 63) // 64) * 2 * D, device=x.device, dtype=torch.float32)
    dx = torch.empty_like(x)
    d_add = torch.empty_like(x) if yout is not None else None
    args = (_p(x), _p(g), _p(n_valid), R, D, _p(gamma), _p(beta), _p(mean), _p(invstd), float(slope), _p(scratch), _p(dgb),
            _p(dx), _p(yout), _p(d_add))
    return args, dgb, dx, d_add, (g, scratch)


class _BNLReLUFn(torch.autograd.Function):
    @staticmethod
    def forward(ctx, x, n_valid, gamma, beta, running_mean, running_var, eps, momentum, slope, training, nbt=None,
                addend=None, ext=None):
        _dev(x, n_valid, gamma, beta, addend)
        x = _f32c(x)
        if addend is not None:
            addend = _f32c(addend)
            if addend.shape != x.shape:
                raise RuntimeError("bn_lrelu: the residual addend must have the shape of the input")
        if not training:
            raise RuntimeError("masked BatchNorm is a training-mode op; use nn.BatchNorm1d in eval mode")
# ... 56 lines not shown
    nbt = bn.num_batches_tracked if (bn.training and bn.track_running_stats) else None
    return _BNLReLUFn.apply(x, n_valid, bn.weight, bn.bias, bn.running_mean, bn.running_var, bn.eps,
                            bn.momentum if bn.momentum is not None else 0.0, slope, bn.training, nbt, addend,
                            bn_stats_of(x))


class _BNLazyFn(torch.autograd.Function):

    @staticmethod
    def forward(ctx, x, n_valid, gamma, beta, mean, invstd, slope):
        y = torch.empty_like(x)
        ctx.save_for_backward(x, n_valid, gamma, beta, mean, invstd)
        ctx.slope = float(slope)
        return y

    @staticmethod
    def backward(ctx, g):
        x, n_valid, gamma, beta, mean, invstd = ctx.saved_tensors
        args, dgb, dx, _, _keep = _bn_bwd_problem(x, g, n_valid, gamma, beta, mean, invstd, ctx.slope, None)
        check(lib().mvk_bn_lrelu_bwd(*args, _stream()))
        D = x.shape[1]
        return dx, None, dgb[D:], dgb[:D], None, None, None


XF_KMAX = 512


def bn_lrelu_linear(x, n_valid, bn, slope, W, stats_n_valid=None, bn_out=None):
    fin = getattr(bn_stats_of(x), "finished", None)
    R, Kd = x.shape
    if (fin is None or not BN_FOLD or _SYNC_BN["group"] is not None or not x.is_cuda or x.dtype != torch.float32
            or not x.is_contiguous() or W.dtype != torch.float32 or not W.is_contiguous() or W.shape[1] != Kd
            or W.shape[0] <= 32 or Kd > XF_KMAX or Kd % 4 != 0 or R == 0 or not slope > 0):
        return None
    mean, invstd = fin
    lazy = _BNLazyFn.apply(x, n_valid, bn.weight, bn.bias, mean, invstd, float(slope))
    xf = {"raw": x.detach(), "mean": mean, "invstd": invstd, "gamma": bn.weight.detach(), "beta": bn.bias.detach(),
          "slope": float(slope), "n_valid": n_valid, "lazy": lazy}
    return linear(lazy, W, stats_n_valid=stats_n_valid, bn=bn_out, _a_transform=xf), lazy


class _BNLReLUPairFn(torch.autograd.Function):

    @staticmethod
    def forward(ctx, xa, xb, n_valid, ga, ba, rma, rva, gb, bb, rmb, rvb, cfg_a, cfg_b, nbt_a, nbt_b, ext_a, ext_b):
        from ._lib import BnFwdProblem
        _dev(xa, xb, n_valid, ga, ba, gb, bb)
        xa, xb = _f32c(xa), _f32c(xb)
        if xa.shape[0] != xb.shape[0]:
            raise RuntimeError("bn_lrelu_pair: the two inputs differ in rows")
        (args_a, ya, mean_a, is_a, _ka), (args_b, yb, mean_b, is_b, _kb) = [
            _bn_fwd_problem("bn_lrelu_pair", x, n_valid, g, b, rm, rv, cfg, nbt, None, ext)
            for x, g, b, rm, rv, cfg, nbt, ext in ((xa, ga, ba, rma, rva, cfg_a, nbt_a, ext_a),
                                                   (xb, gb, bb, rmb, rvb, cfg_b, nbt_b, ext_b))]
        check(lib().mvk_bn_lrelu_fwd_pair(C.byref(BnFwdProblem(*args_a)), C.byref(BnFwdProblem(*args_b)), _stream()))
        ctx.save_for_backward(xa, xb, n_valid, ga, ba, gb, bb, mean_a, is_a, mean_b, is_b)
        ctx.slopes = (float(cfg_a[2]), float(cfg_b[2]))
        ctx.set_materialize_grads(False)
        return ya, yb

    @staticmethod
    def backward(ctx, g_a, g_b):
        from ._lib import BnBwdProblem
        xa, xb, n_valid, ga, ba, gb, bb, mean_a, is_a, mean_b, is_b = ctx.saved_tensors
        (args_a, dgb_a, dx_a, _, _ka), (args_b, dgb_b, dx_b, _, _kb) = [
            _bn_bwd_problem(x, g if g is not None else torch.zeros_like(x), n_valid, gam, bet, mean, istd, slope, None)
            for x, g, gam, bet, mean, istd, slope in ((xa, g_a, ga, ba, mean_a, is_a, ctx.slopes[0]),
                                                      (xb, g_b, gb, bb, mean_b, is_b, ctx.slopes[1]))]
        check(lib().mvk_bn_lrelu_bwd_pair(C.byref(BnBwdProblem(*args_a)), C.byref(BnBwdProblem(*args_b)), _stream()))
        Da, Db = xa.shape[1], xb.shape[1]
        return (dx_a, dx_b, None, dgb_a[Da:], dgb_a[:Da], None, None, dgb_b[Db:], dgb_b[:Db], None, None, None, None, None,
                None, None, None)


def bn_lrelu_pair(xa, bn_a, slope_a, xb, bn_b, slope_b, n_valid):
    def unpack(bn):
        nbt = bn.num_batches_tracked if (bn.training and bn.track_running_stats) else None
        return nbt, (bn.eps, bn.momentum if bn.momentum is not None else 0.0)
    if not (bn_a.training and bn_b.training):
        raise RuntimeError("masked BatchNorm is a training-mode op; use nn.BatchNorm1d in eval mode")
    if _SYNC_BN["group"] is not None:
        return _sync_bn_lrelu(xa, n_valid, bn_a, slope_a, None), _sync_bn_lrelu(xb, n_valid, bn_b, slope_b, None)
    nbt_a, (eps_a, mom_a) = unpack(bn_a)
    nbt_b, (eps_b, mom_b) = unpack(bn_b)
    return _BNLReLUPairFn.apply(xa, xb, n_valid, bn_a.weight, bn_a.bias, bn_a.running_mean, bn_a.running_var,
                                bn_b.weight, bn_b.bias, bn_b.running_mean, bn_b.running_var,
                                (eps_a, mom_a, slope_a), (eps_b, mom_b, slope_b), nbt_a, nbt_b,
                                bn_stats_of(xa), bn_stats_of(xb))


class _AddLReLUFn(torch.autograd.Function):
    @staticmethod
    def forward(ctx, a, b, slope):
        _dev(a, b)
        a, b = _f32c(a), _f32c(b)
        y = torch.empty_like(a)
        check(lib().mvk_add_lrelu_fwd(_p(a), _p(b), a.numel(), float(slope), _p(y), _stream()))
        ctx.save_for_backward(y)
        ctx.slope = float(slope)
        return y

    @staticmethod
    def backward(ctx, g):
        (y,) = ctx.saved_tensors
        g = _f32c(g)
        d = torch.empty_like(y)
        check(lib().mvk_add_lrelu_bwd(_p(y), _p(g), y.numel(), ctx.slope, _p(d), _stream()))
        return d, d.clone(), None


def _bias_grad(y):
    split_arena_prepare(y.device)
    if lib().mvk_gemm_split_ordered():
        return torch.empty((y.shape[1],), device=y.device, dtype=torch.float32)
    return torch.zeros((y.shape[1],), device=y.device, dtype=torch.float32)


class _BiasLReLUFn(torch.autograd.Function):
    @staticmethod
    def forward(ctx, x, bias, slope):
        _dev(x, bias)
        x, bias = _f32c(x), _f32c(bias)
        y = torch.empty_like(x)
        check(lib().mvk_bias_lrelu_fwd(_p(x), _p(bias), x.shape[0], x.shape[1], float(slope), _p(y), _stream()))
        ctx.save_for_backward(y)
        ctx.slope = float(slope)
        return y

    @staticmethod
    def backward(ctx, g):
        (y,) = ctx.saved_tensors
        g = _f32c(g)
        dx = torch.empty_like(y)
        db = _bias_grad(y)
        check(lib().mvk_bias_lrelu_bwd(_p(y), _p(g), y.shape[0], y.shape[1], ctx.slope, _p(dx), _p(db), _stream()))
        return dx, db, None


def bias_lrelu(x, bias, slope=0.1):
    if x.dim() != 2 or bias.dim() != 1 or bias.shape[0] != x.shape[1]:
        raise RuntimeError("bias_lrelu: x [R,C] and bias [C] expected")
    if not slope > 0:
        raise ValueError("bias_lrelu: slope must be positive")
    return _BiasLReLUFn.apply(x, bias, slope)


class _LinearBiasActFn(torch.autograd.Function):

    @staticmethod
    def forward(ctx, x, W, bias, slope):
        _dev(x, W, bias)
        x, W, bias = _f32c(x), _f32c(W), _f32c(bias)
        y = torch.empty((x.shape[0], W.shape[0]), device=x.device, dtype=torch.float32)
        if x.shape[0] > 0:
            check(lib().mvk_gemm_f32_bias_act(_p(x), _p(W), _p(y), x.shape[0], W.shape[0], x.shape[1], 1, _p(bias),
                                              float(slope), _stream()))
        ctx.save_for_backward(x, W, y)
        ctx.slope = float(slope)
        return y

    @staticmethod
    def backward(ctx, g):
        x, W, y = ctx.saved_tensors
        g = _f32c(g)
        d = torch.empty_like(y)
        db = _bias_grad(y)
        check(lib().mvk_bias_lrelu_bwd(_p(y), _p(g), y.shape[0], y.shape[1], ctx.slope, _p(d), _p(db), _stream()))
        dx = gemm(d, W) if ctx.needs_input_grad[0] else None
        dW = _dw_gemm(d, x, target=W) if ctx.needs_input_grad[1] else None
        return dx, dW, db, None


def linear_bias_lrelu(x, W, bias, slope=0.1):
    if x.dim() != 2 or bias.dim() != 1 or bias.shape[0] != W.shape[0] or W.shape[1] != x.shape[1]:
        raise RuntimeError("linear_bias_lrelu: x [R,K], W [C,K] and bias [C] expected")
    if not slope > 0:
        raise ValueError("linear_bias_lrelu: slope must be positive")
    return _LinearBiasActFn.apply(x, W, bias, slope)


def add_lrelu(a, b, slope=0.1):
    if a.shape != b.shape:
        raise RuntimeError("add_lrelu: shapes differ")
    return _AddLReLUFn.apply(a, b, slope)



class _MaxPoolFn(torch.autograd.Function):

    @staticmethod
    def forward(ctx, x, inds, passthrough=False):
        _dev(x, inds)
        x = _f32c(x)
        ctx.rev = reverse_for(inds) if is_deterministic() else None
        inds, i64 = _idx(inds)
        Nq, H = inds.shape
        out = torch.empty((Nq, x.shape[1]), device=x.device, dtype=torch.float32)
        arg = torch.empty((Nq, x.shape[1]), device=x.device, dtype=torch.int32)
        check(lib().mvk_max_pool_fwd(_p(x), x.shape[0], x.shape[1], _p(inds), i64, Nq, H, _p(out), _p(arg), _stream()))
        ctx.save_for_backward(inds, arg)
        ctx.ns, ctx.c = x.shape[0], x.shape[1]
        ctx.set_materialize_grads(False)
        return out, (x.view_as(x) if passthrough else None)

    @staticmethod
    def backward(ctx, g, g_alias=None):
        inds, arg = ctx.saved_tensors
        if g is None:
            return g_alias, None, None
        g = _f32c(g)
        if is_deterministic():
            rev = ctx.rev
            if rev is not None and rev.shape[0] >= ctx.ns:
                base = g_alias if (g_alias is not None and g_alias.shape == (ctx.ns, ctx.c)) else None
                dx = torch.empty((ctx.ns, ctx.c), device=g.device, dtype=torch.float32)
                check(lib().mvk_max_pool_bwd_gather(_p(g), _p(arg), _p(inds), int(inds.dtype == torch.int64), inds.shape[1],
                                                    inds.shape[0], _p(rev), rev.shape[1], ctx.ns, ctx.c,
                                                    _p(_f32c(base)) if base is not None else None, _p(dx), _stream()))
                if g_alias is not None and base is None:
                    dx = dx + g_alias
                return dx, None, None
            _no_reverse_list("a max_pool matrix")
        if (g_alias is not None and g_alias.dtype == torch.float32 and g_alias.is_contiguous()
                and g_alias.shape == (ctx.ns, ctx.c) and _accumulate_in_place_ok(g_alias)):
            dx = g_alias
        else:
            dx = _zeros((ctx.ns, ctx.c), g.device)
        check(lib().mvk_max_pool_bwd(_p(g), _p(arg), _p(inds), int(inds.dtype == torch.int64), inds.shape[0],
                                     inds.shape[1], ctx.ns, g.shape[1], _p(dx), _stream()))
        if g_alias is not None and dx is not g_alias:
            dx = dx + g_alias
        return dx, None, None


class _GatherRowsFn(torch.autograd.Function):
    @staticmethod
    def forward(ctx, x, inds2d):
        _dev(x, inds2d)
        x = _f32c(x)
        ctx.rev = reverse_for(inds2d, first_column=True) if is_deterministic() else None
        inds2d, i64 = _idx(inds2d)
        Nq = inds2d.shape[0]
        stride = inds2d.shape[1] if inds2d.dim() == 2 else 1
        out = torch.empty((Nq, x.shape[1]), device=x.device, dtype=torch.float32)
        check(lib().mvk_gather_rows_fwd(_p(x), x.shape[0], x.shape[1], _p(inds2d), i64, Nq, stride, _p(out), _stream()))
        ctx.save_for_backward(inds2d)
        ctx.ns, ctx.stride = x.shape[0], stride
        return out

    @staticmethod
    def backward(ctx, g):
        (inds2d,) = ctx.saved_tensors
        if not (g.dtype == torch.float32 and g.dim() == 2 and g.stride(1) == 1 and g.stride(0) >= g.shape[1]):
            g = _f32c(g)
        if is_deterministic():
            rev = ctx.rev
            if rev is not None and rev.shape[0] >= ctx.ns:
                return gather_sum_rows(g, rev[:ctx.ns]), None
            _no_reverse_list("a closest_pool / upsampling matrix")
        dx = _zeros((ctx.ns, g.shape[1]), g.device)
        check(lib().mvk_gather_rows_bwd_ld(_p(g), g.stride(0), _p(inds2d), int(inds2d.dtype == torch.int64),
                                           inds2d.shape[0], ctx.stride, ctx.ns, g.shape[1], _p(dx), _stream()))
        return dx, None


class _UpsampleCatFn(torch.autograd.Function):

    @staticmethod
    def forward(ctx, x, inds2d, skip):
        _dev(x, inds2d, skip)
        x, skip = _f32c(x), _f32c(skip)
        ctx.rev = reverse_for(inds2d, first_column=True) if is_deterministic() else None
        inds2d, i64 = _idx(inds2d)
        Nq = inds2d.shape[0]
        if skip.shape[0] != Nq:
            raise RuntimeError("upsample_cat: the skip features and the upsampling indices differ in length")
        stride = inds2d.shape[1] if inds2d.dim() == 2 else 1
        C1, C2 = x.shape[1], skip.shape[1]
        out = torch.empty((Nq, C1 + C2), device=x.device, dtype=torch.float32)
        check(lib().mvk_gather_rows_cat_fwd(_p(x), x.shape[0], C1, _p(inds2d), i64, Nq, stride, _p(skip), C2, _p(out),
                                            _stream()))
        ctx.save_for_backward(inds2d)
        ctx.ns, ctx.stride, ctx.c1 = x.shape[0], stride, C1
        return out

    @staticmethod
    def backward(ctx, g):
        (inds2d,) = ctx.saved_tensors
        g = _f32c(g)
        c2 = g.shape[1] - ctx.c1
        if is_deterministic():
            rev = ctx.rev
            if rev is not None and rev.shape[0] >= ctx.ns:
                dx = gather_sum_rows(g[:, :ctx.c1], rev[:ctx.ns]) if ctx.needs_input_grad[0] else None
                return dx, None, (g[:, ctx.c1:].contiguous() if ctx.needs_input_grad[2] else None)
            _no_reverse_list("a closest_pool / upsampling matrix")
        dx = _zeros((ctx.ns, ctx.c1), g.device) if ctx.needs_input_grad[0] else None
        d_skip = torch.empty((g.shape[0], c2), device=g.device, dtype=torch.float32) if ctx.needs_input_grad[2] else None
        check(lib().mvk_gather_rows_cat_bwd(_p(g), _p(inds2d), int(inds2d.dtype == torch.int64), inds2d.shape[0],
                                            ctx.stride, ctx.ns, ctx.c1, c2, _p(dx), _p(d_skip), _stream()))
        return dx, None, d_skip


class _UpsampleCatLinearFn(torch.autograd.Function):

    @staticmethod
    def forward(ctx, x, inds2d, skip, W, stats_n_valid, finish=None):
        _dev(x, inds2d, skip, W)
        x, skip = _f32c(x), _f32c(skip)
        ctx.rev = reverse_for(inds2d, first_column=True) if is_deterministic() else None
        inds2d, i64 = _idx(inds2d)
        Nq = inds2d.shape[0]
        if skip.shape[0] != Nq:
            raise RuntimeError("upsample_cat_linear: the skip features and the upsampling indices differ in length")
        stride = inds2d.shape[1] if inds2d.dim() == 2 else 1
        C1, C2 = x.shape[1], skip.shape[1]
        cat = torch.empty((Nq, C1 + C2), device=x.device, dtype=torch.float32)
        check(lib().mvk_gather_rows_cat_fwd(_p(x), x.shape[0], C1, _p(inds2d), i64, Nq, stride, _p(skip), C2, _p(cat),
                                            _stream()))
        ctx.set_materialize_grads(False)
        ctx.save_for_backward(cat, W, inds2d)
        ctx.dims = (x.shape[0], C1, C2, stride, i64)
        y, st = _product(cat, W, transB=True, stats_n_valid=stats_n_valid, finish=finish)
        if st is not None:
            ctx.mark_non_differentiable(st.partials)
        return y, st

    @staticmethod
    def backward(ctx, g, g_st=None):
        cat, W, inds2d = ctx.saved_tensors
        ns, C1, C2, stride, i64 = ctx.dims
        g = _f32c(g)
        M, N, Kd = cat.shape[0], C1 + C2, W.shape[0]
        split_arena_prepare(g.device)
        if is_deterministic() and M > 0:
            rev = ctx.rev
            if rev is not None and rev.shape[0] >= ns:
                dx = gemm_ldb(gather_sum_rows(g, rev[:ns]), W, 0, C1, N) if ctx.needs_input_grad[0] else None
                d_skip = gemm_ldb(g, W, C1, C2, N) if ctx.needs_input_grad[2] else None
                dW = _dw_gemm(g, cat, target=W) if ctx.needs_input_grad[3] else None
                return dx, None, d_skip, dW, None, None
            _no_reverse_list("a closest_pool / upsampling matrix")
        dx = _zeros((ns, C1), g.device)
        split = gemm_plan(M, N, Kd, None, False)[0] if M > 0 else 1
        d_skip = _split_out((M, C2), g.device, split)
        if M > 0:
            check(lib().mvk_gemm_f32_scatter_cat(_p(g), _p(W), M, N, Kd, _p(inds2d), i64, stride, ns, C1, _p(dx),
                                                 _p(d_skip), _stream()))
        dW = _dw_gemm(g, cat, target=W) if ctx.needs_input_grad[3] else None
        return (dx if ctx.needs_input_grad[0] else None), None, (d_skip if ctx.needs_input_grad[2] else None), dW, None, None


def upsample_cat_linear(x, inds, skip, W, stats_n_valid=None, bn=None):
    y, st = _UpsampleCatLinearFn.apply(x, inds, skip, W, stats_n_valid,
                                       bn if stats_n_valid is not None and _finishable(bn) else None)
    if st is not None:
        y._mvk_bn_stats = st
    return y


def upsample_cat(x, inds, skip):
    return _UpsampleCatFn.apply(x, inds, skip)


def max_pool(x, inds, passthrough=False):
    out, alias = _MaxPoolFn.apply(x, inds, passthrough)
    return (out, alias) if passthrough else out


def closest_pool(x, inds):
    return _GatherRowsFn.apply(x, inds)



import numpy as _np

_WS = {}


def _workspace(tag, nbytes, device):
    key = (tag, device.index)
    buf = _WS.get(key)
    if buf is None or buf.numel() < nbytes:
        buf = torch.empty(int(nbytes * 1.25) + 1024, dtype=torch.uint8, device=device)
        _WS[key] = buf
    return buf


def _lens_host(lens):
    if isinstance(lens, torch.Tensor):
        lens = lens.detach().cpu().numpy()
    return _np.ascontiguousarray(lens, dtype=_np.int32)


def grid_subsample_batch(points, lens, features=None, labels=None, dl=0.1, max_p=0, rotations=None):
    _dev(points, features, labels)
    points = _f32c(points)
    lens_h = _lens_host(lens)
    N, B = points.shape[0], int(lens_h.shape[0])
    fdim = ldim = 0
    if features is not None:
        features = _f32c(features)
        fdim = features.shape[1]
    if labels is not None:
        labels = labels.to(torch.int32).contiguous()
        if labels.dim() == 1:
            labels = labels.unsqueeze(1)
        ldim = labels.shape[1]
    ws = _workspace("sub", lib().mvk_grid_subsample_workspace(N, B, fdim, ldim), points.device)
    out_pts = torch.empty((max(N, 1), 3), device=points.device, dtype=torch.float32)
    out_f = torch.empty((max(N, 1), fdim), device=points.device, dtype=torch.float32) if fdim else None
    out_l = torch.empty((max(N, 1), ldim), device=points.device, dtype=torch.int32) if ldim else None
    out_lens = torch.empty((B,), device=points.device, dtype=torch.int32)
    out_lens_h = _np.empty((B,), _np.int32)
    tail = (_p(features), fdim, _p(labels), ldim, float(dl), int(max_p), _p(out_pts), _p(out_f), _p(out_l),
            _p(out_lens), out_lens_h.ctypes.data_as(C.c_void_p), _p(ws), ws.numel(), _stream())
    if rotations is None:
        check(lib().mvk_grid_subsample_batch(_p(points), N, lens_h.ctypes.data_as(C.c_void_p), B, *tail))
    else:
        rot = _np.ascontiguousarray(rotations, dtype=_np.float32)
        if rot.shape != (B, 3, 3):
            raise RuntimeError("grid_subsample_batch: rotations must be [B,3,3]")
        check(lib().mvk_grid_subsample_batch_oriented(_p(points), N, lens_h.ctypes.data_as(C.c_void_p), B,
                                                      rot.ctypes.data_as(C.c_void_p), *tail))
    M = int(out_lens_h.sum())
    res = [out_pts[:M], out_lens_h]
    if fdim:
        res.append(out_f[:M])
    if ldim:
        res.append(out_l[:M])
    return tuple(res)


_NB_GRID = {}


def radius_neighbors_batch(queries, supports, q_lens, s_lens, radius, limit=None, status=None, reuse_grid=False):
    _dev(queries, supports)
    q, s = _f32c(queries), _f32c(supports)
    ql, sl = _lens_host(q_lens), _lens_host(s_lens)
    if ql.shape[0] != sl.shape[0]:
        raise RuntimeError("Wrong number of batch elements: different for queries and supports ")
    Nq, Ns, B = q.shape[0], s.shape[0], int(ql.shape[0])
    ws = _workspace("nb", lib().mvk_radius_neighbors_workspace(Nq, Ns, B), q.device)
    args = (_p(q), Nq, _p(s), Ns, ql.ctypes.data_as(C.c_void_p), sl.ctypes.data_as(C.c_void_p), B, float(radius))
    if status is not None:
        if limit is None:
            raise RuntimeError("radius_neighbors_batch: the enqueue-only mode needs a column limit")
        _dev(status)
        width = int(limit)
        out = torch.empty((Nq, width), device=q.device, dtype=torch.int32)
        reuse = bool(reuse_grid) and _NB_GRID.get(q.device.index) == ws.data_ptr()
        if width > 0 and Nq > 0:
            check(lib().mvk_radius_neighbors_enqueue(*args, _p(out), width, _p(status), int(reuse), _p(ws),
                                                     ws.numel(), _stream()))
            _NB_GRID[q.device.index] = ws.data_ptr()
        return out
    _NB_GRID.pop(q.device.index, None)
    if limit is None:
        w = C.c_int(0)
        check(lib().mvk_radius_neighbors_batch(*args, None, 0, C.byref(w), _p(ws), ws.numel(), _stream()))
        width = int(w.value)
    else:
        width = int(limit)
    out = torch.empty((Nq, width), device=q.device, dtype=torch.int32)
    if width > 0 and Nq > 0:
        w = C.c_int(0)
        check(lib().mvk_radius_neighbors_batch(*args, _p(out), width, C.byref(w), _p(ws), ws.numel(), _stream()))
        if int(w.value) < width:
            out = out[:, :int(w.value)].contiguous()
    return out


def grid_subsample_dev(points, lens_dev, dl, out_points, out_lens_dev, status, rotations_dev=None,
                       total_out=None, pad_value=1e6):
    _dev(points, lens_dev, out_points, out_lens_dev, status, rotations_dev, total_out)
    points = _f32c(points)
    cap_in, B = points.shape[0], int(lens_dev.shape[0])
    if not out_points.is_contiguous() or out_points.dtype != torch.float32:
        raise RuntimeError("grid_subsample_dev: out_points must be a contiguous float32 [cap,3] tensor")
    ws = _workspace("sub", lib().mvk_grid_subsample_workspace(cap_in, B, 0, 0), points.device)
    check(lib().mvk_grid_subsample_batch_dev(_p(points), cap_in, _p(lens_dev), B, _p(rotations_dev), float(dl),
                                             _p(out_points), out_points.shape[0], float(pad_value),
                                             _p(out_lens_dev), _p(total_out), _p(status), _p(ws), ws.numel(), _stream()))


def radius_neighbors_dev(queries, supports, q_lens_dev, s_lens_dev, radius, out, shadow, status, reuse_grid=False,
                         rev=None, rev_counts=None, rev_status=None):
    _dev(queries, supports, q_lens_dev, s_lens_dev, out, status, rev, rev_counts, rev_status)
    q, s = _f32c(queries), _f32c(supports)
    if out.dtype != torch.int32 or not out.is_contiguous() or out.shape[0] != q.shape[0]:
        raise RuntimeError("radius_neighbors_dev: out must be a contiguous int32 [Nq_cap, width] tensor")
    B = int(q_lens_dev.shape[0])
    ws = _workspace("nb", lib().mvk_radius_neighbors_workspace(q.shape[0], s.shape[0], B), q.device)
    if rev is not None:
        if (rev.dtype != torch.int32 or not rev.is_contiguous() or rev.dim() != 2 or rev.shape[0] < s.shape[0]
                or rev_counts is None or rev_counts.dtype != torch.int32 or rev_counts.numel() < s.shape[0] or rev_status is None):
            raise RuntimeError("radius_neighbors_dev: rev must be a contiguous int32 [>= Ns_cap, Hr] matrix with int32 "
                               "counters [>= Ns_cap] and a status word")
        check(lib().mvk_radius_neighbors_dev_rev(_p(q), q.shape[0], _p(s), s.shape[0], _p(q_lens_dev), _p(s_lens_dev), B,
                                                 float(radius), _p(out), out.shape[1], int(shadow), _p(status),
                                                 int(bool(reuse_grid)), _p(ws), ws.numel(), _p(rev), rev.shape[1],
                                                 _p(rev_counts), _p(rev_status), _stream()))
    else:
        check(lib().mvk_radius_neighbors_dev(_p(q), q.shape[0], _p(s), s.shape[0], _p(q_lens_dev), _p(s_lens_dev), B,
                                             float(radius), _p(out), out.shape[1], int(shadow), _p(status),
                                             int(bool(reuse_grid)), _p(ws), ws.numel(), _stream()))
    _NB_GRID.pop(q.device.index, None)


REG_MANY = CONSTANTS["MVK_REG_MANY"]
REV_MANY = CONSTANTS["MVK_REV_MANY"]


def reverse_finish_many(lists, status=None):
    from ._lib import RevList
    for i0 in range(0, len(lists), REV_MANY):
        chunk = lists[i0:i0 + REV_MANY]
        arr = (RevList * len(chunk))()
        for k, (rev, counts, rows, shadow) in enumerate(chunk):
            _dev(rev, counts, status)
            arr[k] = RevList(_p(rev), _p(counts), _p(status), int(rows), int(rev.shape[1]), int(shadow))
        check(lib().mvk_reverse_finish_many(arr, len(chunk), _stream()))


def neighbors_cell_order(Nq, Ns, B, out=None, s_lens_dev=None, device=None):
    dev = out.device if out is not None else (s_lens_dev.device if s_lens_dev is not None else device)
    if out is None:
        out = torch.empty((Ns,), device=dev, dtype=torch.int32)
    _dev(out, s_lens_dev)
    if out.dtype != torch.int32 or not out.is_contiguous() or out.dim() != 1 or out.shape[0] < Ns:
        raise RuntimeError("neighbors_cell_order: out must be a contiguous int32 vector of at least Ns entries")
    ws = _workspace("nb", lib().mvk_radius_neighbors_workspace(Nq, Ns, B), dev)
    check(lib().mvk_neighbors_cell_order(Ns, B, _p(s_lens_dev), _p(out), out.shape[0], _p(ws), ws.numel(), _stream()))
    return out


_REV_COUNTS = {}
_REV_COUNTS_RETIRED = []
REVERSE_DX = os.environ.get("MVK_REVERSE_DX", "1") == "1"


def _rev_counts(n, device):
    key = device.index
    buf = _REV_COUNTS.get(key)
    if buf is None or buf.numel() < n:
        if torch.cuda.is_current_stream_capturing():
            raise RuntimeError("ops.reverse_neighbors: the counter buffer of this device does not exist yet (or is too "
                               "small) and cannot be created inside a graph capture; build one batch eagerly first")
        if buf is not None:
            _REV_COUNTS_RETIRED.append(buf)
        buf = torch.zeros(max(int(n), 1 << 16), dtype=torch.int32, device=device)
        torch.cuda.current_stream(device).synchronize()
        _REV_COUNTS[key] = buf
    return buf


REV_MAX_WIDTH = CONSTANTS["MVK_REV_MAX_WIDTH"]


def reverse_width_cap(sort=None):
    return REV_MAX_WIDTH


def reverse_neighbors(idx, Ns, width=None, out=None, status=None, shadow=None, sort=None, first_column=False):
    _dev(idx, out, status)
    idx, i64 = _idx(idx)
    Nq, H = idx.shape[0], idx.shape[1] if idx.dim() == 2 else 0
    stride = H
    if first_column:
        H = min(H, 1)
    Ns = int(Ns)
    shadow = Nq if shadow is None else int(shadow)
    dev = idx.device
    counts = _rev_counts(Ns, dev)
    do_sort = int(is_deterministic() if sort is None else bool(sort))

    def run(dst, w, st):
        check(lib().mvk_reverse_neighbors(_p(idx), i64, Nq, H, max(stride, H), Ns, _p(dst), int(w), shadow, do_sort,
                                          _p(counts), _p(st), _stream()))

    if out is not None:
        if out.dtype != torch.int32 or not out.is_contiguous() or out.dim() != 2 or out.shape[0] < Ns:
            raise RuntimeError("reverse_neighbors: out must be a contiguous int32 [>= Ns, width] matrix")
        run(out, out.shape[1], status)
        return out
    if width is not None:
        rev = torch.empty((Ns, max(int(width), 1)), device=dev, dtype=torch.int32)
        run(rev, rev.shape[1], status)
        return rev
    st = torch.zeros(2, dtype=torch.int32, device=dev)
    cap = reverse_width_cap(do_sort)
    w = max(8, min(cap, 2 * H + 8))
    rev = torch.empty((Ns, w), device=dev, dtype=torch.int32)
    run(rev, w, st)
    longest, ovf = (int(v) for v in st.cpu())
    if ovf:
        if longest > cap:
            raise RuntimeError("reverse_neighbors: a support has %d reverse neighbours (> %d)" % (longest, cap))
        rev = torch.empty((Ns, longest), device=dev, dtype=torch.int32)
        run(rev, longest, None)
        return rev
    return rev[:, :max(longest, 1)].contiguous()


_REVERSES = collections.OrderedDict()
_REVERSES_KEPT = 256


def _rev_key(inds, first):
    return (inds.device.index, inds.data_ptr(), tuple(inds.shape), inds.dtype, bool(first))


def remember_reverse(inds, rev, first_column=False):
    key = _rev_key(inds, first_column)
    if len(_REVERSES) >= 16:
        for k in [k for k, e in _REVERSES.items() if e[0]() is None]:
            del _REVERSES[k]
    _REVERSES[key] = (weakref.ref(inds), rev)
    _REVERSES.move_to_end(key)
    while len(_REVERSES) > _REVERSES_KEPT:
        _REVERSES.popitem(last=False)


def reverse_for(inds, first_column=False):
    if not (torch.is_tensor(inds) and inds.is_cuda):
        return None
    e = _REVERSES.get(_rev_key(inds, first_column))
    return e[1] if (e is not None and e[0]() is inds) else None


_DET_WARNED = set()
# ... 1672 lines not shown
```

Measured before the change: 5.458 million points/s.

## Split decoder upsample-cat-linear into coarse GEMM plus gathered row addend

The decoder's upsample+concat+linear no longer materializes the concatenated matrix. Its forward runs two GEMMs: first the coarse features times their weight columns at coarse resolution, then the skip features times the remaining columns with the coarse result gathered per row as an epilogue addend. The backward reduces the gradient to coarse rows first, then computes dx and d_skip in a paired NN launch and writes dW as column slabs via new ldc/ldb GEMM entry points. This cuts gather/concat traffic and runs the C1 part at coarse row count, at the cost of an extra intermediate, more launches and a new add-epilogue kernel variant.

```diff
diff --git a/enhancing-3d-point-cloud-segmentation-using-multi-modal-fusion-with-2d-images_amd/_lib.py b/enhancing-3d-point-cloud-segmentation-using-multi-modal-fusion-with-2d-images_amd/_lib.py
--- a/enhancing-3d-point-cloud-segmentation-using-multi-modal-fusion-with-2d-images_amd/_lib.py
+++ b/enhancing-3d-point-cloud-segmentation-using-multi-modal-fusion-with-2d-images_amd/_lib.py
@@ -8,6 +8,7 @@
 SCENE_HEADER_PATH = os.path.join(_HERE, "..", "include", "mvkpconv_scene.h")
 TRAIN_HEADER_PATH = os.path.join(_HERE, "..", "include", "mvkpconv_train.h")
 SPHERE_HEADER_PATH = os.path.join(_HERE, "..", "include", "mvkpconv_sphere.h")
+DECODER_HEADER_PATH = os.path.join(_HERE, "..", "include", "mvkpconv_decoder.h")
 
 CTYPES = {"int": C.c_int, "int32_t": C.c_int32, "int64_t": C.c_int64, "float": C.c_float, "double": C.c_double,
           "const char*": C.c_char_p}
@@ -139,6 +140,12 @@
         or SPHERE_CONSTANTS.keys() & (CONSTANTS.keys() | SCENE_CONSTANTS.keys() | TRAIN_CONSTANTS.keys())):
     raise ValueError("mvkpconv_sphere.h: it may declare neither a struct nor a name of the other three headers")
 _SPHERE_PROTOTYPES = _bind(SPHERE_FUNCTIONS, {})[1]
+
+DECODER_FUNCTIONS, _decoder_structs, _decoder_constants = parse_header(_read_header(DECODER_HEADER_PATH, "mvkpconv_decoder.h"))
+if (_decoder_structs or _decoder_constants
+        or DECODER_FUNCTIONS.keys() & (FUNCTIONS.keys() | SCENE_FUNCTIONS.keys() | TRAIN_FUNCTIONS.keys() | SPHERE_FUNCTIONS.keys())):
+    raise ValueError("mvkpconv_decoder.h: it may declare neither a struct, a constant nor a name of the other four headers")
+_DECODER_PROTOTYPES = _bind(DECODER_FUNCTIONS, {})[1]
 BnFwdProblem, BnBwdProblem = _CLASSES["mvk_bn_fwd_problem"], _CLASSES["mvk_bn_bwd_problem"]
 BnFinish, ATransform = _CLASSES["mvk_bn_finish"], _CLASSES["mvk_a_transform"]
 RevList, RegLayer = _CLASSES["mvk_rev_list"], _CLASSES["mvk_reg_layer"]
@@ -174,7 +181,7 @@
                 "no CPU fallback for the MV-KPConv hot path." % LIB_PATH)
         l = C.CDLL(LIB_PATH)
         for name, (res, args) in list(_PROTOTYPES.items()) + list(_SCENE_PROTOTYPES.items()) + list(_TRAIN_PROTOTYPES.items()) \
-                + list(_SPHERE_PROTOTYPES.items()):
+                + list(_SPHERE_PROTOTYPES.items()) + list(_DECODER_PROTOTYPES.items()):
             fn = getattr(l, name)
             fn.restype = res
             fn.argtypes = args
diff --git a/enhancing-3d-point-cloud-segmentation-using-multi-modal-fusion-with-2d-images_amd/build.py b/enhancing-3d-point-cloud-segmentation-using-multi-modal-fusion-with-2d-images_amd/build.py
--- a/enhancing-3d-point-cloud-segmentation-using-multi-modal-fusion-with-2d-images_amd/build.py
+++ b/enhancing-3d-point-cloud-segmentation-using-multi-modal-fusion-with-2d-images_amd/build.py
@@ -53,6 +53,7 @@
     common = [os.path.join(CSRC, "common.h"), os.path.join(CSRC, "blockscan.h"), os.path.join(CSRC, "compact.h"),
               os.path.join(CSRC, "pn2_rows.h"), os.path.join(CSRC, "unproject.h"), os.path.join(CSRC, "select_frames.h"),
               os.path.join(CSRC, "knn_core.h"), os.path.join(HERE, "..", "include", "mvkpconv_sphere.h"),
+              os.path.join(HERE, "..", "include", "mvkpconv_decoder.h"),
               os.path.join(HERE, "..", "include", "mvkpconv.h"), os.path.join(HERE, "..", "include", "mvkpconv_scene.h"),
               os.path.join(HERE, "..", "include", "mvkpconv_train.h"),
               os.path.join(HERE, "..", "include", "mvk_prime_list.h"), os.path.abspath(__file__)]
diff --git a/enhancing-3d-point-cloud-segmentation-using-multi-modal-fusion-with-2d-images_amd/csrc/gemm.hip b/enhancing-3d-point-cloud-segmentation-using-multi-modal-fusion-with-2d-images_amd/csrc/gemm.hip
--- a/enhancing-3d-point-cloud-segmentation-using-multi-modal-fusion-with-2d-images_amd/csrc/gemm.hip
+++ b/enhancing-3d-point-cloud-segmentation-using-multi-modal-fusion-with-2d-images_amd/csrc/gemm.hip
@@ -1,9 +1,11 @@
 #include <stdlib.h>
 
 #include <mutex>
+#include <vector>
 #include <type_traits>
 
 #include "common.h"
+#include "../../include/mvkpconv_decoder.h"
 
 namespace {
 
@@ -215,11 +217,16 @@
   float ax_slope;
   const int32_t* ax_nvalid;
   float* ax_out;
+  int64_t ldc;
+  const float* add_src;
+  const void* add_idx;
+  int add_idx64;
+  int64_t add_stride, add_ns;
 };
 
 constexpr int XF_KMAX = 512;
 
-template <bool TA, bool TB, int PM, int QN, int WM, int WN, bool DUAL = false, bool XF = false>
+template <bool TA, bool TB, int PM, int QN, int WM, int WN, bool DUAL = false, bool XF = false, bool ADD = false>
 __device__ __forceinline__ void gemm_body(const GemmArgs& a, const int bx, const int by, const int bz) {
   static_assert(WM * WN == 4, "four waves per workgroup");
   constexpr int TM = 16 * PM * WM, TN = 16 * QN * WN;
@@ -402,6 +409,27 @@
   }
 
   const int ci = lane & 15, g4 = (lane >> 4) * 4;
+  if constexpr (ADD) {
+    if (a.add_src && (a.det_ws || bz == 0)) {
+#pragma unroll
+      for (int p = 0; p < PM; ++p)
+#pragma unroll
+        for (int r = 0; r < 4; ++r) {
+          const int64_t row = m0 + ra + 16 * p + g4 + r;
+          if (row < a.M) {
+            const int j = a.add_idx64 ? load_idx<true>(a.add_idx, row * a.add_stride, a.add_ns)
+                                      : load_idx<false>(a.add_idx, row * a.add_stride, a.add_ns);
+            if (j >= 0) {
+#pragma unroll
+              for (int q = 0; q < QN; ++q) {
+                const int64_t col = n0 + rb + 16 * q + ci;
+                if (col < a.N) acc[p][q][r] += a.add_src[(int64_t)j * a.N + col];
+              }
+            }
+          }
+        }
+    }
+  }
 #pragma unroll
   for (int q = 0; q < QN; ++q) {
     const int64_t col = n0 + rb + 16 * q + ci;
@@ -426,7 +454,7 @@
               }
               continue;
             }
-            float* c = a.C + row * a.N + col;
+            float* c = a.C + row * a.ldc + col;
             if (a.atomic_out)
               atomicAdd(c, acc[p][q][r]);
             else if (a.accumulate)
@@ -605,13 +633,19 @@
   gemm_body<false, TB, PM, 1, 1, 4, false, true>(a, blockIdx.x, blockIdx.y, blockIdx.z);
 }
 
+template <int PM, int QN, int WM, int WN>
+__global__ __launch_bounds__(256) void gemm_f32_mfma_add(const GemmArgs a) {
+  gemm_body<false, true, PM, QN, WM, WN, false, false, true>(a, blockIdx.x, blockIdx.y, blockIdx.z);
+}
+
 template <bool TA, bool TB, int PM, int QN, int WM, int WN>
-__global__ __launch_bounds__(256) void gemm_f32_mfma_pair(const GemmArgs a0, const GemmArgs a1, int gx0, int gz0, int gz1) {
+__global__ __launch_bounds__(256) void gemm_f32_mfma_pair(const GemmArgs a0, const GemmArgs a1, int gx0, int gy0, int gy1,
+                                                          int gz0, int gz1) {
   if ((int)blockIdx.x < gx0) {
-    if ((int)blockIdx.z >= gz0) return;
+    if ((int)blockIdx.z >= gz0 || (int)blockIdx.y >= gy0) return;
     gemm_body<TA, TB, PM, QN, WM, WN>(a0, blockIdx.x, blockIdx.y, blockIdx.z);
   } else {
-    if ((int)blockIdx.z >= gz1) return;
+    if ((int)blockIdx.z >= gz1 || (int)blockIdx.y >= gy1) return;
     gemm_body<TA, TB, PM, QN, WM, WN>(a1, blockIdx.x - gx0, blockIdx.y, blockIdx.z);
   }
 }
@@ -784,15 +818,17 @@
 }
 
 template <bool TA, bool TB, int PM>
-void launch_pair_one(dim3 grid, hipStream_t st, const GemmArgs& a0, const GemmArgs& a1, int gx0, int gz0, int gz1) {
-  hipLaunchKernelGGL((gemm_f32_mfma_pair<TA, TB, PM, 1, 1, 4>), grid, dim3(256), 0, st, a0, a1, gx0, gz0, gz1);
+void launch_pair_one(dim3 grid, hipStream_t st, const GemmArgs& a0, const GemmArgs& a1, int gx0, int gy0, int gy1, int gz0,
+                     int gz1) {
+  hipLaunchKernelGGL((gemm_f32_mfma_pair<TA, TB, PM, 1, 1, 4>), grid, dim3(256), 0, st, a0, a1, gx0, gy0, gy1, gz0, gz1);
 }
 
 template <bool TA, bool TB>
-bool launch_pair_cfg(const Plan& p, dim3 grid, hipStream_t st, const GemmArgs& a0, const GemmArgs& a1, int gx0, int gz0, int gz1) {
+bool launch_pair_cfg(const Plan& p, dim3 grid, hipStream_t st, const GemmArgs& a0, const GemmArgs& a1, int gx0, int gy0, int gy1,
+                     int gz0, int gz1) {
   if (p.qn != 1) return false;
-  if (p.pm == 2) return launch_pair_one<TA, TB, 2>(grid, st, a0, a1, gx0, gz0, gz1), true;
-  if (p.pm == 4) return launch_pair_one<TA, TB, 4>(grid, st, a0, a1, gx0, gz0, gz1), true;
+  if (p.pm == 2) return launch_pair_one<TA, TB, 2>(grid, st, a0, a1, gx0, gy0, gy1, gz0, gz1), true;
+  if (p.pm == 4) return launch_pair_one<TA, TB, 4>(grid, st, a0, a1, gx0, gy0, gy1, gz0, gz1), true;
   return false;
 }
 
@@ -820,7 +856,7 @@
 GemmArgs make_args(const float* A, const float* B, float* C, int64_t M, int64_t N, int64_t Kd, int64_t lda, int64_t ldb,
                    KSplit ks) {
   GemmArgs a{};
-  a.A = A; a.B = B; a.C = C; a.M = M; a.N = N; a.Kd = Kd;
+  a.A = A; a.B = B; a.C = C; a.M = M; a.N = N; a.Kd = Kd; a.ldc = N;
   a.lda = lda; a.ldb = ldb; a.vecA = vec_width(A, lda); a.vecB = vec_width(B, ldb);
   a.k_per_split = ks.k_per_split; a.atomic_out = ks.n > 1; a.det_nsplit = ks.n;
   a.act_slope = 1.f; a.ax_slope = 1.f; a.vecA2 = 1; a.vecB2 = 1; a.seg_shift = -1;
@@ -847,6 +883,13 @@
   float* rest;
 };
 
+struct RowAddend {
+  const float* src;
+  const void* idx;
+  int idx64;
+  int64_t stride, ns;
+};
+
 struct GemmOpts {
   int accumulate = 0, split_k = 0;
   float* bn_part = nullptr;
@@ -856,6 +899,8 @@
   const ScatterOut* scatter = nullptr;
   int seg_shift = -1;
   int64_t seg_extra = 0, ldb = 0, lda = 0;
+  int64_t ldc = 0;
+  const RowAddend* add = nullptr;
   const mvk_bn_finish* fin = nullptr;
   const mvk_a_transform* ax = nullptr;
 };
@@ -866,7 +911,10 @@
   if (M == 0 || N == 0) return 0;
   hipStream_t st = (hipStream_t)stream;
   MVK_REQUIRE(!(o.bn_part && (o.accumulate || Kd == 0)), "gemm: BatchNorm statistics need a plain store of a non-empty product");
+  MVK_REQUIRE(o.ldc <= 0 || o.ldc >= N, "gemm: ldc < N");
+  const int64_t ldc = o.ldc > 0 ? o.ldc : N;
   if (Kd == 0) {
+    MVK_REQUIRE(ldc == N && !o.add, "gemm: an empty reduction into a column window or with an addend");
     if (!o.accumulate && o.split_k <= 1) MVK_CHECK_HIP(hipMemsetAsync(C, 0, sizeof(float) * M * N, st));
     return 0;
   }
@@ -875,14 +923,14 @@
   const KSplit ks = clamp_split(Kd, p.split);
   const int64_t lda = o.lda > 0 ? o.lda : (transA ? M : Kd);
   if (cdiv64(M, p.tm()) >= 65536) {
-    MVK_REQUIRE(!o.bn_part && !o.fin && !o.ax && !o.scatter && o.seg_shift < 0 && ks.n < 65536, "gemm: grid too large");
+    MVK_REQUIRE(!o.bn_part && !o.fin && !o.ax && !o.scatter && !o.add && o.seg_shift < 0 && ks.n < 65536, "gemm: grid too large");
     constexpr int64_t CHUNK = 15 * 65536;
     GemmOpts oc = o;
     oc.split_k = ks.n;
     oc.lda = lda;
     for (int64_t m0 = 0; m0 < M; m0 += CHUNK) {
       const int64_t mc = M - m0 < CHUNK ? M - m0 : CHUNK;
-      if (int e = gemm_run(A + (transA ? m0 : m0 * lda), B, C + m0 * N, mc, N, Kd, transA, transB, oc, stream)) return e;
+      if (int e = gemm_run(A + (transA ? m0 : m0 * lda), B, C + m0 * ldc, mc, N, Kd, transA, transB, oc, stream)) return e;
     }
     return 0;
   }
@@ -892,7 +940,7 @@
     a.vecB = ((uintptr_t)B % 16 == 0 && o.seg_extra % 4 == 0) ? 4 : 1;
   }
   a.accumulate = o.accumulate; a.bn_part = o.bn_part; a.n_valid = o.n_valid; a.bias = o.bias; a.act_slope = o.act_slope;
-  a.seg_shift = o.seg_shift; a.seg_extra = o.seg_extra;
+  a.seg_shift = o.seg_shift; a.seg_extra = o.seg_extra; a.ldc = ldc;
   if (o.scatter) {
     a.sc_idx = o.scatter->idx; a.sc_idx64 = o.scatter->idx64; a.sc_c1 = o.scatter->c1; a.sc_stride = o.scatter->stride;
     a.sc_ns = o.scatter->ns; a.sc_dst = o.scatter->dst; a.sc_rest = o.scatter->rest;
@@ -903,13 +951,25 @@
   MVK_REQUIRE(!(o.bn_part && ks.n > 1 && !a.det_ws), "gemm: BatchNorm statistics of a split product need the ordered reduction");
   if (int e = set_finish(a, o.fin, grid.y)) return e;
   if (const mvk_a_transform* ax = o.ax) {
-    MVK_REQUIRE(!transA && transB && !p.narrow && p.qn == 1 && (p.pm == 2 || p.pm == 4) && ks.k_per_split <= XF_KMAX && !o.scatter &&
+    MVK_REQUIRE(!transA && transB && !p.narrow && p.qn == 1 && (p.pm == 2 || p.pm == 4) && ks.k_per_split <= XF_KMAX && !o.scatter && !o.add &&
                     o.seg_shift < 0 && ax->mean && ax->invstd && ax->gamma && ax->beta && ax->slope > 0.f,
                 "gemm: the operand transform needs an NT product of more than 32 columns with k-ranges <= %d", XF_KMAX);
     a.ax_mean = ax->mean; a.ax_invstd = ax->invstd; a.ax_gamma = ax->gamma; a.ax_beta = ax->beta; a.ax_slope = ax->slope;
     a.ax_nvalid = ax->n_valid; a.ax_out = ax->out;
     if (p.pm == 2) hipLaunchKernelGGL((gemm_f32_mfma_xf<true, 2>), grid, dim3(256), 0, st, a);
     else hipLaunchKernelGGL((gemm_f32_mfma_xf<true, 4>), grid, dim3(256), 0, st, a);
+    MVK_CHECK_HIP(hipGetLastError());
+    return 0;
+  }
+  if (const RowAddend* ad = o.add) {
+    MVK_REQUIRE(!transA && transB && !o.scatter && !o.accumulate && o.seg_shift < 0 && ad->src && ad->idx && ad->stride >= 1 && ad->ns >= 0,
+                "gemm: the row-gathered addend needs an NT product with a plain store, a source and an index");
+    a.add_src = ad->src; a.add_idx = ad->idx; a.add_idx64 = ad->idx64; a.add_stride = ad->stride; a.add_ns = ad->ns;
+    if (p.narrow && p.pm == 1 && p.qn == 1) hipLaunchKernelGGL((gemm_f32_mfma_add<1, 1, 4, 1>), grid, dim3(256), 0, st, a);
+    else if (p.narrow && p.pm == 1 && p.qn == 2) hipLaunchKernelGGL((gemm_f32_mfma_add<1, 2, 4, 1>), grid, dim3(256), 0, st, a);
+    else if (!p.narrow && p.pm == 2 && p.qn == 1) hipLaunchKernelGGL((gemm_f32_mfma_add<2, 1, 1, 4>), grid, dim3(256), 0, st, a);
+    else if (!p.narrow && p.pm == 4 && p.qn == 1) hipLaunchKernelGGL((gemm_f32_mfma_add<4, 1, 1, 4>), grid, dim3(256), 0, st, a);
+    else MVK_REQUIRE(false, "gemm: no addend kernel for plan pm=%d qn=%d narrow=%d", p.pm, p.qn, p.narrow);
     MVK_CHECK_HIP(hipGetLastError());
     return 0;
   }
@@ -948,11 +1008,18 @@
   if (int e = set_finish(a0, fin0, gy)) return e;
   if (int e = set_finish(a1, fin1, gy)) return e;
   dim3 grid((unsigned)(gx0 + gx1), (unsigned)gy, (unsigned)(s0.n > s1.n ? s0.n : s1.n));
-  const bool ok = transB ? launch_pair_cfg<false, true>(p0, grid, st, a0, a1, gx0, s0.n, s1.n)
-                         : launch_pair_cfg<false, false>(p0, grid, st, a0, a1, gx0, s0.n, s1.n);
+  const bool ok = transB ? launch_pair_cfg<false, true>(p0, grid, st, a0, a1, gx0, (int)gy, (int)gy, s0.n, s1.n)
+                         : launch_pair_cfg<false, false>(p0, grid, st, a0, a1, gx0, (int)gy, (int)gy, s0.n, s1.n);
   MVK_REQUIRE(ok, "gemm pair: no kernel for plan pm=%d", p0.pm);
   MVK_CHECK_HIP(hipGetLastError());
   return 0;
+}
+
+bool nn_pair_plans(int64_t M0, int64_t N0, int64_t M1, int64_t N1, int64_t Kd, Plan& p0, Plan& p1) {
+  if (M0 <= 0 || N0 <= 0 || M1 <= 0 || N1 <= 0 || Kd <= 0) return false;
+  p0 = plan_gemm(M0, N0, Kd, 0, false);
+  p1 = plan_gemm(M1, N1, Kd, 0, false);
+  return !p0.narrow && !p1.narrow && p0.pm == p1.pm && p0.qn == 1 && p1.qn == 1 && (p0.pm == 2 || p0.pm == 4);
 }
 
 }
@@ -1087,6 +1154,56 @@
   return gemm_run(A, B, C, M, N, Kd, 0, 0, o, stream);
 }
 
+extern "C" int mvk_gemm_f32_nt_ldb_add(const float* A, const float* B, int64_t col0, int64_t ldb, float* C, int64_t M, int64_t N,
+                                       int64_t Kd, const float* add_src, const void* add_idx, int add_idx64,
+                                       int64_t add_stride, int64_t add_ns, float* bn_part, const int32_t* n_valid,
+                                       const void* fin , void* stream) {
+  MVK_REQUIRE(M > 0 && N > 0 && Kd > 0 && col0 >= 0 && ldb >= col0 + Kd, "gemm nt_ldb_add: empty product or a column block outside B");
+  MVK_REQUIRE((add_src == nullptr) == (add_idx == nullptr), "gemm nt_ldb_add: the addend needs its source and its index");
+  const RowAddend ad{add_src, add_idx, add_idx64, add_stride, add_ns};
+  GemmOpts o; o.ldb = ldb; o.bn_part = bn_part; o.n_valid = n_valid; o.fin = (const mvk_bn_finish*)fin; o.add = add_src ? &ad : nullptr;
+  return gemm_run(A, B + col0, C, M, N, Kd, 0, 1, o, stream);
+}
+
+extern "C" int mvk_gemm_f32_tn_ldc(const float* A, const float* B, float* C, int64_t M, int64_t N, int64_t Kd, int64_t ldc,
+                                   void* stream) {
+  MVK_REQUIRE(ldc >= N && Kd > 0, "gemm tn_ldc: ldc < N or an empty reduction");
+  GemmOpts o; o.ldc = ldc;
+  return gemm_run(A, B, C, M, N, Kd, 1, 0, o, stream);
+}
+
+extern "C" int mvk_gemm_f32_nn_pair_plan(int64_t M0, int64_t N0, int64_t M1, int64_t N1, int64_t Kd, int* out ) {
+  MVK_REQUIRE(M0 >= 0 && N0 >= 0 && M1 >= 0 && N1 >= 0 && Kd >= 0 && out, "gemm nn pair plan: bad arguments");
+  out[0] = out[1] = out[2] = 0;
+  Plan p0, p1;
+  if (!nn_pair_plans(M0, N0, M1, N1, Kd, p0, p1)) return 0;
+  out[0] = 1;
+  out[1] = clamp_split(Kd, p0.split).n;
+  out[2] = clamp_split(Kd, p1.split).n;
+  return 0;
+}
+
+extern "C" int mvk_gemm_f32_nn_pair(const float* A0, const float* B0, float* C0, int64_t M0, int64_t N0, const float* A1,
+                                    const float* B1, float* C1, int64_t M1, int64_t N1, int64_t Kd, int64_t ldb, void* stream) {
+  Plan p0, p1;
+  MVK_REQUIRE(nn_pair_plans(M0, N0, M1, N1, Kd, p0, p1) && ldb >= N0 && ldb >= N1,
+              "gemm nn pair: the two products do not share a tile shape (ask mvk_gemm_f32_nn_pair_plan first)");
+  hipStream_t st = (hipStream_t)stream;
+  const KSplit s0 = clamp_split(Kd, p0.split), s1 = clamp_split(Kd, p1.split);
+  GemmArgs a0 = make_args(A0, B0, C0, M0, N0, Kd, Kd, ldb, s0);
+  GemmArgs a1 = make_args(A1, B1, C1, M1, N1, Kd, Kd, ldb, s1);
+  const int64_t tm = p0.tm(), tn = p0.tn(), gy0 = cdiv64(M0, tm), gy1 = cdiv64(M1, tm);
+  MVK_REQUIRE(gy0 < 65536 && gy1 < 65536 && s0.n < 65536 && s1.n < 65536, "gemm: grid too large");
+  const int gx0 = (int)cdiv64(N0, tn), gx1 = (int)cdiv64(N1, tn);
+  MVK_ORDERED(make_ordered(st, a0, s0.n, gx0, gy0, tm, tn));
+  MVK_ORDERED(make_ordered(st, a1, s1.n, gx1, gy1, tm, tn));
+  dim3 grid((unsigned)(gx0 + gx1), (unsigned)(gy0 > gy1 ? gy0 : gy1), (unsigned)(s0.n > s1.n ? s0.n : s1.n));
+  const bool ok = launch_pair_cfg<false, false>(p0, grid, st, a0, a1, gx0, (int)gy0, (int)gy1, s0.n, s1.n);
+  MVK_REQUIRE(ok, "gemm nn pair: no kernel for plan pm=%d", p0.pm);
+  MVK_CHECK_HIP(hipGetLastError());
+  return 0;
+}
+
 extern "C" int mvk_gemm_f32_scatter_cat(const float* A, const float* B, int64_t M, int64_t N, int64_t Kd, const void* idx,
                                         int idx64, int64_t idx_stride, int64_t Ns, int c1, float* d_x, float* d_skip,
                                         void* stream) {
@@ -1102,6 +1219,12 @@
   float* C;
   int64_t M, N, Kd;
 };
+struct MvkGemmProblemLdc {
+  const float* A;
+  const float* B;
+  float* C;
+  int64_t M, N, Kd, ldc;
+};
 
 extern "C" int64_t mvk_gemm_group_entry_bytes(void) { return (int64_t)sizeof(GroupEntry); }
 
@@ -1128,11 +1251,11 @@
   return grouped_split_at(M, N, Kd, e >= 0 ? e : GROUP_KTILES_MIN);
 }
 
-extern "C" int mvk_gemm_f32_tn_grouped_plan(const void* problems, int n, void* table_host, int* n_narrow,
-                                            int64_t* wgs_narrow, int64_t* wgs_wide, int32_t* splits ,
-                                            void* stream ) {
+extern "C" int mvk_gemm_f32_tn_grouped_plan_ldc(const void* problems, int n, void* table_host, int* n_narrow,
+                                                int64_t* wgs_narrow, int64_t* wgs_wide, int32_t* splits ,
+                                                void* stream ) {
   MVK_REQUIRE(n >= 0 && problems && table_host && n_narrow && wgs_narrow && wgs_wide && splits, "grouped gemm: bad arguments");
-  const MvkGemmProblem* pr = (const MvkGemmProblem*)problems;
+  const MvkGemmProblemLdc* pr = (const MvkGemmProblemLdc*)problems;
   GroupEntry* tab = (GroupEntry*)table_host;
   int nn = 0;
   for (int i = 0; i < n; ++i) nn += pr[i].N <= 32 ? 1 : 0;
@@ -1147,14 +1270,16 @@
     ktiles = t < GROUP_KTILES_MIN ? GROUP_KTILES_MIN : (t > GROUP_KTILES_MAX ? GROUP_KTILES_MAX : (int)t);
   }
   for (int i = 0; i < n; ++i) {
-    const MvkGemmProblem& q = pr[i];
+    const MvkGemmProblemLdc& q = pr[i];
     MVK_REQUIRE(q.M > 0 && q.N > 0 && q.Kd > 0 && q.A && q.B && q.C, "grouped gemm: empty problem %d", i);
     const bool narrow = q.N <= 32;
     MVK_REQUIRE(!narrow || q.N > 16, "grouped gemm: outputs of <= 16 columns are not grouped");
+    MVK_REQUIRE(q.ldc >= q.N, "grouped gemm: ldc < N in problem %d", i);
     const KSplit ks = clamp_split(q.Kd, grouped_split_at(q.M, q.N, q.Kd, ktiles));
     const int split = ks.n;
     GroupEntry e{};
     e.args = make_args(q.A, q.B, q.C, q.M, q.N, q.Kd, q.M, q.N, ks);
+    e.args.ldc = q.ldc;
     const int64_t tm = narrow ? 64 : 16 * group_wide_pm(), tn = narrow ? 32 : 64;
     e.gx = (int)cdiv64(q.N, tn);
     e.gy = (int)cdiv64(q.M, tm);
@@ -1177,6 +1302,17 @@
   *wgs_narrow = wn;
   *wgs_wide = ww;
   return 0;
+}
+
+extern "C" int mvk_gemm_f32_tn_grouped_plan(const void* problems, int n, void* table_host, int* n_narrow,
+                                            int64_t* wgs_narrow, int64_t* wgs_wide, int32_t* splits ,
+                                            void* stream) {
+  MVK_REQUIRE(n >= 0 && problems, "grouped gemm: bad arguments");
+  const MvkGemmProblem* pr = (const MvkGemmProblem*)problems;
+  std::vector<MvkGemmProblemLdc> v((size_t)n);
+  for (int i = 0; i < n; ++i) v[i] = MvkGemmProblemLdc{pr[i].A, pr[i].B, pr[i].C, pr[i].M, pr[i].N, pr[i].Kd, pr[i].N};
+  static const MvkGemmProblemLdc none{};
+  return mvk_gemm_f32_tn_grouped_plan_ldc(n > 0 ? v.data() : &none, n, table_host, n_narrow, wgs_narrow, wgs_wide, splits, stream);
 }
 
 extern "C" int mvk_gemm_f32_tn_grouped(const void* table_dev, int n, int n_narrow, int64_t wgs_narrow, int64_t wgs_wide,
diff --git a/enhancing-3d-point-cloud-segmentation-using-multi-modal-fusion-with-2d-images_amd/ops.py b/enhancing-3d-point-cloud-segmentation-using-multi-modal-fusion-with-2d-images_amd/ops.py
--- a/enhancing-3d-point-cloud-segmentation-using-multi-modal-fusion-with-2d-images_amd/ops.py
+++ b/enhancing-3d-point-cloud-segmentation-using-multi-modal-fusion-with-2d-images_amd/ops.py
@@ -464,9 +464,9 @@
         return
     if stream is None or stream == torch.cuda.current_stream():
         return _flush_deferred(items)
-    for (A, B, _, _, _) in items:
-        A.record_stream(stream)
-        B.record_stream(stream)
+    for it in items:
+        it[0].record_stream(stream)
+        it[1].record_stream(stream)
     with torch.cuda.stream(stream):
         _flush_deferred(items)
 
@@ -486,14 +486,15 @@
     import numpy as np
     dev = items[0][0].device
     n = len(items)
-    prob = np.zeros(n, dtype=np.dtype([("A", "<u8"), ("B", "<u8"), ("C", "<u8"), ("M", "<i8"), ("N", "<i8"), ("Kd", "<i8")]))
-    for i, (A, B, out_ptr, _, storage) in enumerate(items):
+    prob = np.zeros(n, dtype=np.dtype([("A", "<u8"), ("B", "<u8"), ("C", "<u8"), ("M", "<i8"), ("N", "<i8"), ("Kd", "<i8"),
+                                       ("ldc", "<i8")]))
+    for i, (A, B, out_ptr, _, storage, ldc) in enumerate(items):
         if _storage_use_count(storage) < 2:
             raise RuntimeError("defer_weight_grads: a deferred weight-gradient result (%d x %d) was consumed before the "
                                "grouped launch computed it; was the backward run on parameters that already hold a "
                                ".grad, or with hooks that copy gradients? Run it without the scope (MVK_DEFER_DW=0)"
                                % (A.shape[1], B.shape[1]))
-        prob[i] = (A.data_ptr(), B.data_ptr(), out_ptr, A.shape[1], B.shape[1], A.shape[0])
+        prob[i] = (A.data_ptr(), B.data_ptr(), out_ptr, A.shape[1], B.shape[1], A.shape[0], ldc)
     slots = _defer_slots(dev)
     if torch.cuda.is_current_stream_capturing():
         if len(slots) <= 2:
@@ -507,7 +508,7 @@
             slot["event"].synchronize()
     nn, wn, ww = C.c_int(0), C.c_int64(0), C.c_int64(0)
     splits = np.zeros(n, np.int32)
-    check(lib().mvk_gemm_f32_tn_grouped_plan(prob.ctypes.data_as(C.c_void_p), n, C.c_void_p(slot["host"].data_ptr()),
+    check(lib().mvk_gemm_f32_tn_grouped_plan_ldc(prob.ctypes.data_as(C.c_void_p), n, C.c_void_p(slot["host"].data_ptr()),
                                              C.byref(nn), C.byref(wn), C.byref(ww), splits.ctypes.data_as(C.c_void_p),
                                              _stream()))
     for i, item in enumerate(items):
@@ -524,10 +525,15 @@
 
 def _accumulate_in_place_ok(t):
     if _DEFER["on"] and _DEFER["items"]:
-        st = t.untyped_storage().data_ptr()
+        if not t.is_contiguous():
+            return False
+        lo = t.data_ptr()
+        hi = lo + t.numel() * t.element_size()
         for it in _DEFER["items"]:
-            if it[0].untyped_storage().data_ptr() == st or it[1].untyped_storage().data_ptr() == st:
-                return False
+            for op in (it[0], it[1]):
+                a = op.data_ptr()
+                if a < hi and lo < a + op.numel() * op.element_size():
+                    return False
     return True
 
 
@@ -547,11 +553,46 @@
             and not lib().mvk_gemm_split_ordered()
         out = (_zeros((A.shape[1], B.shape[1]), A.device) if zeroed
                else torch.empty((A.shape[1], B.shape[1]), device=A.device, dtype=torch.float32))
-        _DEFER["items"].append((A, B, out.data_ptr(), zeroed, out.untyped_storage()))
+        _DEFER["items"].append((A, B, out.data_ptr(), zeroed, out.untyped_storage(), B.shape[1]))
         if leaf is not None:
             _DEFER["leaves"].add(id(leaf))
         return out
     return gemm(A, B, transA=True, transB=transB)
+
+
+def _dw_gemm_slabs(slabs, target=None):
+    leaf = target if (target is not None and target.is_leaf) else None
+    defer = _DEFER["on"] and _HAS_USE_COUNT
+    if _DEFER["on"] and leaf is not None:
+        if id(leaf) in _DEFER["leaves"]:
+            raise RuntimeError("defer_weight_grads: the same parameter receives two weight gradients inside one scope "
+                               "(shared weights): run this backward without the scope (MVK_DEFER_DW=0)")
+        if leaf.grad is not None:
+            defer = False
+    slabs = [(_f32c(A), _f32c(B)) for A, B in slabs]
+    dev, M = slabs[0][0].device, slabs[0][0].shape[1]
+    ld = sum(B.shape[1] for _, B in slabs)
+    grouped = [defer and B.shape[1] > 16 for _, B in slabs]
+    if sum(grouped) + len(_DEFER["items"]) > _DW_MAX:
+        grouped = [False] * len(slabs)
+    split_arena_prepare(dev)
+    ordered = bool(lib().mvk_gemm_split_ordered())
+    zeroed = not ordered and any(
+        (lib().mvk_gemm_f32_tn_grouped_split(M, B.shape[1], A.shape[0]) if gr else gemm_plan(M, B.shape[1], A.shape[0])[0]) > 1
+        for (A, B), gr in zip(slabs, grouped))
+    out = _zeros((M, ld), dev) if zeroed else torch.empty((M, ld), device=dev, dtype=torch.float32)
+    storage = out.untyped_storage() if any(grouped) else None
+    col0 = 0
+    for (A, B), gr in zip(slabs, grouped):
+        ptr = out.data_ptr() + 4 * col0
+        if gr:
+            _DEFER["items"].append((A, B, ptr, zeroed, storage, ld))
+        else:
+            check(lib().mvk_gemm_f32_tn_ldc(_p(A), _p(B), C.c_void_p(ptr), M, B.shape[1], A.shape[0], ld, _stream()))
+        col0 += B.shape[1]
+    if any(grouped) and leaf is not None:
+        _DEFER["leaves"].add(id(leaf))
+    return out
 
 
 
@@ -1214,6 +1255,29 @@
         return dx, None, d_skip
 
 
+DECODER_SPLIT = os.environ.get("MVK_DECODER_SPLIT", "1") != "0"
+
+
+def _nt_ldb_add(A, W, col0, Kd, addend=None, stats_n_valid=None, finish=None):
+    M, N = A.shape[0], W.shape[0]
+    split_arena_prepare(A.device)
+    stats_ok = stats_n_valid is not None and M <= _STATS_EPILOGUE_ROWS
+    if finish is None:
+        stats_ok = stats_ok and M > bn_single_launch_rows(N)
+    split, rows = gemm_plan(M, N, Kd, None, stats_ok)
+    out = _split_out((M, N), A.device, split)
+    part = torch.empty(((M + rows - 1) // rows, 2, N), device=A.device, dtype=torch.float32) if rows > 0 else None
+    fin = done = None
+    if finish is not None and part is not None:
+        fin, done = _fin_struct(finish, N, A.device)
+    src, idx, i64, stride = addend if addend is not None else (None, None, 0, 1)
+    check(lib().mvk_gemm_f32_nt_ldb_add(_p(A), _p(W), int(col0), W.shape[1], _p(out), M, N, int(Kd), _p(src), _p(idx), int(i64),
+                                        int(stride), src.shape[0] if src is not None else 0, _p(part),
+                                        _p(stats_n_valid) if part is not None else None,
+                                        C.byref(fin) if fin is not None else None, _stream()))
+    return out, (BnStats(part, rows, done) if part is not None else None)
+
+
 class _UpsampleCatLinearFn(torch.autograd.Function):
 
     @staticmethod
@@ -1227,6 +1291,19 @@
             raise RuntimeError("upsample_cat_linear: the skip features and the upsampling indices differ in length")
         stride = inds2d.shape[1] if inds2d.dim() == 2 else 1
         C1, C2 = x.shape[1], skip.shape[1]
+        ctx.split_form = bool(DECODER_SPLIT and Nq > 0 and x.shape[0] > 0 and C1 > 0 and C2 > 0 and W.shape[0] > 0)
+        if ctx.split_form:
+            W = _f32c(W)
+            if W.shape[1] != C1 + C2:
+                raise RuntimeError("upsample_cat_linear: the weight has %d input columns, the inputs %d + %d" % (W.shape[1], C1, C2))
+            ctx.set_materialize_grads(False)
+            ctx.save_for_backward(x, skip, W, inds2d)
+            ctx.dims = (x.shape[0], C1, C2, stride, i64)
+            Yc, _ = _nt_ldb_add(x, W, 0, C1)
+            y, st = _nt_ldb_add(skip, W, C1, C2, (Yc, inds2d, i64, stride), stats_n_valid, finish)
+            if st is not None:
+                ctx.mark_non_differentiable(st.partials)
+            return y, st
         cat = torch.empty((Nq, C1 + C2), device=x.device, dtype=torch.float32)
         check(lib().mvk_gather_rows_cat_fwd(_p(x), x.shape[0], C1, _p(inds2d), i64, Nq, stride, _p(skip), C2, _p(cat),
                                             _stream()))
@@ -1239,7 +1316,47 @@
         return y, st
 
     @staticmethod
+    def _backward_split(ctx, g):
+        x, skip, W, inds2d = ctx.saved_tensors
+        ns, C1, C2, stride, i64 = ctx.dims
+        need_x, need_skip, need_w = ctx.needs_input_grad[0], ctx.needs_input_grad[2], ctx.needs_input_grad[3]
+        g = _f32c(g)
+        Nq, N = g.shape
+        split_arena_prepare(g.device)
+        det = False
+        if is_deterministic():
+            det = ctx.rev is not None and ctx.rev.shape[0] >= ns
+            if not det:
+                _no_reverse_list("a closest_pool / upsampling matrix")
+        Gc = None
+        if need_x or need_w:
+            if det:
+                Gc = gather_sum_rows(g, ctx.rev[:ns])
+            else:
+                Gc = _zeros((ns, N), g.device)
+                check(lib().mvk_gather_rows_bwd_ld(_p(g), N, _p(inds2d), i64, Nq, stride, ns, N, _p(Gc), _stream()))
+        dx = d_skip = None
+        if need_x and need_skip and not det:
+            plan = (C.c_int * 3)()
+            check(lib().mvk_gemm_f32_nn_pair_plan(ns, C1, Nq, C2, N, plan))
+            if plan[0]:
+                dx = _split_out((ns, C1), g.device, plan[1])
+                d_skip = _split_out((Nq, C2), g.device, plan[2])
+                check(lib().mvk_gemm_f32_nn_pair(_p(Gc), _p(W), _p(dx), ns, C1, _p(g), C.c_void_p(W.data_ptr() + 4 * C1),
+                                                 _p(d_skip), Nq, C2, N, C1 + C2, _stream()))
+        if need_x and dx is None:
+            dx = gemm_ldb(Gc, W, 0, C1, C1 + C2)
+        if need_skip and d_skip is None:
+            d_skip = gemm_ldb(g, W, C1, C2, C1 + C2)
+        dW = _dw_gemm_slabs([(Gc, x), (g, skip)], target=W) if need_w else None
+        return dx, None, d_skip, dW, None, None
+
+    @staticmethod
     def backward(ctx, g, g_st=None):
+        if g is None:
+            return None, None, None, None, None, None
+        if ctx.split_form:
+            return _UpsampleCatLinearFn._backward_split(ctx, g)
         cat, W, inds2d = ctx.saved_tensors
         ns, C1, C2, stride, i64 = ctx.dims
         g = _f32c(g)
diff --git a/include/mvkpconv_decoder.h b/include/mvkpconv_decoder.h
--- /dev/null
+++ b/include/mvkpconv_decoder.h
@@ -0,0 +1,28 @@
+#ifndef MVKPCONV_DECODER_H
+#define MVKPCONV_DECODER_H
+
+#include <stdint.h>
+
+#ifdef __cplusplus
+extern "C" {
+#endif
+
+int mvk_gemm_f32_nt_ldb_add(const float* A, const float* B, int64_t col0, int64_t ldb, float* C, int64_t M, int64_t N,
+                            int64_t Kd, const float* add_src, const void* add_idx, int add_idx64, int64_t add_stride,
+                            int64_t add_ns, float* bn_part, const int32_t* n_valid, const void* fin, void* stream);
+
+int mvk_gemm_f32_nn_pair_plan(int64_t M0, int64_t N0, int64_t M1, int64_t N1, int64_t Kd, int* out );
+int mvk_gemm_f32_nn_pair(const float* A0, const float* B0, float* C0, int64_t M0, int64_t N0, const float* A1,
+                         const float* B1, float* C1, int64_t M1, int64_t N1, int64_t Kd, int64_t ldb, void* stream);
+
+int mvk_gemm_f32_tn_ldc(const float* A, const float* B, float* C, int64_t M, int64_t N, int64_t Kd, int64_t ldc,
+                        void* stream);
+
+int mvk_gemm_f32_tn_grouped_plan_ldc(const void* problems, int n, void* table_host, int* n_narrow, int64_t* wgs_narrow,
+                                     int64_t* wgs_wide, int32_t* splits, void* stream);
+
+#ifdef __cplusplus
+}
+#endif
+
+#endif
```

Result: faster. 5.530 million points/s, median of 6 (+1.3%).
